# noway/nzcb-circom

Hardware: AMD Instinct MI355X
Metric: PLONK proofs/sec for nzcp_live (~2^21 constraints) at 1/2/4/8 MI355X (higher is better)
Workload: dtype u32 limbs: BN254 Fr/Fq Montgomery, 8x32-bit and 9x29-bit (MSM, NTT twiddles, quotient); 1 GPU; nzcp_live fullProve: NZCPPubIdentity(1,351,0,4,2,4) witness on the GPU (600560 signals) + PLONK proof, n=2^21, nPublic=3, 2970 inputs; domain_size=2097152, n_public=3, n_constraints=1785813, n_vars=1782570, n_additions=1182010, proofs_per_gpu=140, total_proofs=140, parallelism=batch-shard x1 (no collective), proofs_in_flight_per_gpu=5

## Files before the change

include/nzcb_internal.h:

```cpp
#ifndef NZCB_INTERNAL_H
#define NZCB_INTERNAL_H

#include "nzcb.h"

#ifdef __cplusplus
extern "C" {
#endif

int nzcb_ctx_kernel_stats(nzcb_ctx* ctx, int enable, double out[4]);

int nzcb_debug_guard_check(int device, size_t* checked, int* damaged, nzcb_err* err);
int nzcb_debug_guard_selftest(int device, nzcb_err* err);

#define NZCB_FAULT_QUOTIENT 1
#define NZCB_DEBUG_GENERIC_K 2
#define NZCB_FAULT_LANE_ALLOC 3
int nzcb_debug_inject_fault(nzcb_ctx* ctx, int kind);

int nzcb_debug_f29(int device, int op, const uint32_t* in, size_t count, uint32_t* out, nzcb_err* err);

int nzcb_synth_setup(int power, int n_public, int n_inputs, uint64_t seed, uint32_t n_constraints,
                     const uint8_t* tau, int device, uint8_t** zkey_out, size_t* zkey_len, uint8_t** wtns_out,
                     size_t* wtns_len, nzcb_err* err);
#define NZCB_SYNTH_FREE_PUBLIC 1u
int nzcb_synth_setup_ex(int power, int n_public, int n_inputs, uint64_t seed, uint32_t n_constraints, uint32_t flags,
                        const uint8_t* tau, int device, uint8_t** zkey_out, size_t* zkey_len, uint8_t** wtns_out,
                        size_t* wtns_len, nzcb_err* err);
typedef struct nzcb_engine nzcb_engine;
nzcb_engine* nzcb_engine_create(int device, int max_log_ntt, size_t max_msm_points, nzcb_err* err);
void nzcb_engine_destroy(nzcb_engine* e);
int nzcb_engine_ntt(nzcb_engine* e, const uint8_t* in_lem, uint8_t* out_lem, int log_n, int inverse, nzcb_err* err);
int nzcb_engine_msm(nzcb_engine* e, const uint8_t* bases_lem, const uint8_t* scalars, size_t n, int scalars_mont,
                    uint8_t* out_affine, nzcb_err* err);
int nzcb_engine_ntt_dev(nzcb_engine* e, const void* in, void* out, int log_n, int inverse, nzcb_err* err);
int nzcb_engine_msm_dev(nzcb_engine* e, const void* bases, const void* scalars, size_t n, int scalars_mont,
                        uint8_t* out_affine, nzcb_err* err);
int nzcb_engine_time_ntt(nzcb_engine* e, const void* in, void* out, int log_n, int inverse, int reps, double* ms,
                         nzcb_err* err);
int nzcb_engine_random_fr(nzcb_engine* e, void* dev_out, size_t n, uint64_t seed, nzcb_err* err);
int nzcb_engine_fixed_base(nzcb_engine* e, const void* dev_scalars_mont, size_t n, void* dev_out, nzcb_err* err);
int nzcb_engine_lagrange_basis(nzcb_engine* e, const void* dev_ptau, size_t ptau_n, int log_n, void* dev_out,
                               nzcb_err* err);
int nzcb_engine_time_msm(nzcb_engine* e, const void* bases, const void* scalars, size_t n, int scalars_mont, int reps,
                         double* ms, double* acc_ms, nzcb_err* err);
int nzcb_engine_msm_fixed_dev(nzcb_engine* e, const void* bases, size_t n_table, const void* scalars, size_t n,
                              int scalars_mont, uint8_t* out_affine, nzcb_err* err);
int nzcb_engine_msm_table_dev(nzcb_engine* e, const void* bases, size_t n_table, const void* scalars, size_t n,
                              int scalars_mont, int window, int sparse, int fold, uint8_t* out_affine,
                              nzcb_err* err);
int nzcb_engine_msm_sets_dev(nzcb_engine* e, const void* bases, size_t n_table, const void* const* scalars, int sets,
                             size_t n, int scalars_mont, int sparse, uint8_t* out_affine, nzcb_err* err);
int nzcb_engine_time_msm2(nzcb_engine* e, const void* bases, const void* scalars, size_t n, int scalars_mont,
                          int fixed_base, int reps, double* out, nzcb_err* err);
int nzcb_engine_fr_mul(nzcb_engine* e, const uint8_t* a_lem, const uint8_t* b_lem, uint8_t* out_lem, size_t n,
                       int field_q, nzcb_err* err);

int nzcb_engine_g1_lincomb(int device, const uint8_t* points, const uint8_t* scalars, const uint32_t* group_end,
                           size_t groups, uint8_t* out, nzcb_err* err);
int nzcb_engine_verify_batch(const uint8_t* vk, const uint8_t* proofs, const uint8_t* pubs, size_t pub_stride,
                             int n_public, int count, int transcript_public, int device, const uint8_t* seed,
                             int* valid_out, uint8_t* points_out, int* pairing_checks, nzcb_err* err);
int nzcb_debug_verify_batch_timings(double* ms, int cap);

nzcb_r1cs* nzcb_engine_r1cs_create(const uint8_t* r1cs, size_t len, int device, uint32_t long_row_threshold,
                                   int witness_tile, nzcb_err* err);
int nzcb_debug_r1cs_check_timings(double* ms, int cap);

nzcb_p256_key* nzcb_engine_p256_key_create(const uint8_t pub_xy[64], int device, int window, nzcb_err* err);
#define NZCB_P256_OP_ADD 0
#define NZCB_P256_OP_SUB 1
#define NZCB_P256_OP_MUL 2
#define NZCB_P256_OP_SQR 3
#define NZCB_P256_OP_INV 4
int nzcb_debug_p256_field(int device, int op, int field, const uint8_t* a, const uint8_t* b, size_t count,
                          uint8_t* out, nzcb_err* err);
int nzcb_debug_p256_mul2(nzcb_p256_key* k, const uint8_t* u1, const uint8_t* u2, size_t count, uint8_t* out_xy,
                         nzcb_err* err);
int nzcb_debug_p256_timings(double* ms, int cap);

int nzcb_debug_nzcp_decode_timings(double* ms, int cap);

#ifdef __cplusplus
}
#endif
#endif
```

nzcb-circom_amd/csrc/capi_engine.hip:

```cpp
#include <chrono>
#include <cstring>
#include <map>
#include <memory>
#include <mutex>
#include <vector>

#include "../../include/nzcb_internal.h"
#include "engine.h"
#include "lagrange.h"

namespace nzcb {

Engine::Engine(int dev, int max_log_ntt, size_t max_msm_points) : device(dev) {
  NZ_HIP(hipSetDevice(dev));
  NZ_HIP(hipStreamCreateWithFlags(&stream, hipStreamNonBlocking));
  if (max_log_ntt >= 0) ntt_tables.init(max_log_ntt, stream);
  if (max_msm_points) msm_scratch.init(max_msm_points);
}

Engine::~Engine() {
  if (stream) (void)hipStreamDestroy(stream);
}

void set_err(nzcb_err* err, int code, const char* msg) {
// ... 38 lines not shown
  std::vector<uint8_t> h(kGuardBytes);
  int bad = 0;
  for (auto& r : recs) {
    NZ_HIP(hipMemcpy(h.data(), (uint8_t*)r.first + r.second.bytes, kGuardBytes, hipMemcpyDeviceToHost));
    size_t k = 0;
    while (k < kGuardBytes && h[k] == kGuardByte) k++;
    if (k == kGuardBytes) continue;
    bad++;
    if (report && bad <= 8) {
      char line[160];
      std::snprintf(line, sizeof(line), "%sbuffer %p (%zu bytes, device %d): guard byte %zu overwritten",
                    report->empty() ? "" : "; ", r.first, r.second.bytes, r.second.device, k);
      *report += line;
    }
  }
  if (checked) *checked = recs.size();
  return bad;
}

__global__ void k_guard_poke(uint32_t* p, size_t at) {
  if (threadIdx.x == 0) p[at] = 0;
}

}

using namespace nzcb;

struct nzcb_engine {
  Engine eng;
  nzcb_engine(int d, int l, size_t m) : eng(d, l, m) {}
};

#define NZ_GUARD_BEGIN try {
#define NZ_GUARD_END(err)                                   \
  }                                                         \
  catch (const nzcb::Error& e) {                            \
    set_err(err, e.code, e.what());                         \
    return e.code;                                          \
  }                                                         \
  catch (const std::exception& e) {                         \
    set_err(err, NZCB_ERR_INTERNAL, e.what());              \
    return NZCB_ERR_INTERNAL;                               \
  }

__global__ void fe_mul_kernel_r(const Fr* a, const Fr* b, Fr* o, size_t n) {
  size_t i = (size_t)blockIdx.x * blockDim.x + threadIdx.x;
  if (i < n) o[i] = a[i] * b[i];
}
__global__ void fe_mul_kernel_q(const Fq* a, const Fq* b, Fq* o, size_t n) {
  size_t i = (size_t)blockIdx.x * blockDim.x + threadIdx.x;
  if (i < n) o[i] = a[i] * b[i];
}

__global__ void random_fr_kernel(Fr* out, size_t n, uint64_t seed) {
  size_t i = (size_t)blockIdx.x * blockDim.x + threadIdx.x;
  if (i >= n) return;
  uint64_t x = seed ^ (0x9E3779B97F4A7C15ULL * (i + 1));
  Fr v;
  for (int k = 0; k < 4; k++) {
    x += 0x9E3779B97F4A7C15ULL;
    uint64_t z = x;
    z = (z ^ (z >> 30)) * 0xBF58476D1CE4E5B9ULL;
    z = (z ^ (z >> 27)) * 0x94D049BB133111EBULL;
    z ^= z >> 31;
    v.v[2 * k] = (uint32_t)z;
    v.v[2 * k + 1] = (uint32_t)(z >> 32);
  }
  v.v[7] &= 0x1fffffffu;
  out[i] = to_mont(v);
}

static void affine_out(const G1xyzz& r, uint8_t* out) {
  G1Affine a = xyzz_to_affine(r);
  Fq x = a.is_inf() ? Fq::zero() : from_mont(a.x);
  Fq y = a.is_inf() ? Fq::zero() : from_mont(a.y);
  std::memcpy(out, x.v, 32);
  std::memcpy(out + 32, y.v, 32);
}

extern "C" {

const char* nzcb_version(void) { return "nzcb-mi355x 0.1.0 (gfx950)"; }

int nzcb_device_count(void) {
  int n = 0;
  if (hipGetDeviceCount(&n) != hipSuccess) return 0;
  return n;
}

void nzcb_free(void* p) { std::free(p); }

nzcb_engine* nzcb_engine_create(int device, int max_log_ntt, size_t max_msm_points, nzcb_err* err) {
  try {
    return new nzcb_engine(device, max_log_ntt, max_msm_points);
  } catch (const nzcb::Error& e) {
    set_err(err, e.code, e.what());
  } catch (const std::exception& e) {
    set_err(err, NZCB_ERR_INTERNAL, e.what());
  }
  return nullptr;
}

void nzcb_engine_destroy(nzcb_engine* e) { delete e; }

void* nzcb_dev_alloc(size_t bytes) {
  void* p = nullptr;
  if (hipMalloc(&p, bytes) != hipSuccess) return nullptr;
  return p;
}
void* nzcb_dev_alloc_on(int device, size_t bytes) {
  int cur = 0;
  if (hipGetDevice(&cur) != hipSuccess || hipSetDevice(device) != hipSuccess) return nullptr;
  void* p = nullptr;
  if (hipMalloc(&p, bytes) != hipSuccess) p = nullptr;
  (void)hipSetDevice(cur);
  return p;
}
void nzcb_dev_free(void* p) {
  if (p) (void)hipFree(p);
}
int nzcb_memcpy_h2d(void* dst, const void* src, size_t bytes) {
  return hipMemcpy(dst, src, bytes, hipMemcpyHostToDevice) == hipSuccess ? 0 : NZCB_ERR_HIP;
}
int nzcb_memcpy_d2h(void* dst, const void* src, size_t bytes) {
  return hipMemcpy(dst, src, bytes, hipMemcpyDeviceToHost) == hipSuccess ? 0 : NZCB_ERR_HIP;
}
int nzcb_memcpy_d2d(void* dst, const void* src, size_t bytes) {
  if (hipMemcpyAsync(dst, src, bytes, hipMemcpyDeviceToDevice, nullptr) != hipSuccess) return NZCB_ERR_HIP;
  return hipStreamSynchronize(nullptr) == hipSuccess ? 0 : NZCB_ERR_HIP;
}
int nzcb_memcpy_d2d_async(void* dst, const void* src, size_t bytes, void* stream) {
  return hipMemcpyAsync(dst, src, bytes, hipMemcpyDeviceToDevice, (hipStream_t)stream) == hipSuccess ? 0
                                                                                              : NZCB_ERR_HIP;
}

int nzcb_engine_ntt_dev(nzcb_engine* e, const void* in, void* out, int log_n, int inverse, nzcb_err* err) {
  NZ_GUARD_BEGIN
  Engine& g = e->eng;
  NZ_HIP(hipSetDevice(g.device));
  ntt(g.ntt_tables, (const Fr*)in, (Fr*)out, log_n, inverse != 0, g.stream);
  NZ_HIP(hipStreamSynchronize(g.stream));
  return 0;
  NZ_GUARD_END(err)
}

int nzcb_engine_ntt(nzcb_engine* e, const uint8_t* in_lem, uint8_t* out_lem, int log_n, int inverse, nzcb_err* err) {
  NZ_GUARD_BEGIN
  Engine& g = e->eng;
  NZ_HIP(hipSetDevice(g.device));
  size_t n = size_t(1) << log_n;
  DevBuf<Fr> a(n), b(n);
  NZ_HIP(hipMemcpyAsync(a.p, in_lem, n * 32, hipMemcpyHostToDevice, g.stream));
  ntt(g.ntt_tables, a.p, b.p, log_n, inverse != 0, g.stream);
  NZ_HIP(hipMemcpyAsync(out_lem, b.p, n * 32, hipMemcpyDeviceToHost, g.stream));
  NZ_HIP(hipStreamSynchronize(g.stream));
  return 0;
  NZ_GUARD_END(err)
}

int nzcb_engine_time_ntt(nzcb_engine* e, const void* in, void* out, int log_n, int inverse, int reps, double* ms,
                         nzcb_err* err) {
  NZ_GUARD_BEGIN
  Engine& g = e->eng;
  NZ_HIP(hipSetDevice(g.device));
  hipEvent_t e0, e1;
  NZ_HIP(hipEventCreate(&e0));
  NZ_HIP(hipEventCreate(&e1));
  NZ_HIP(hipEventRecord(e0, g.stream));
  for (int i = 0; i < reps; i++) ntt(g.ntt_tables, (const Fr*)in, (Fr*)out, log_n, inverse != 0, g.stream);
  NZ_HIP(hipEventRecord(e1, g.stream));
  NZ_HIP(hipEventSynchronize(e1));
  float t = 0;
  NZ_HIP(hipEventElapsedTime(&t, e0, e1));
  *ms = t / (reps > 0 ? reps : 1);
  (void)hipEventDestroy(e0);
  (void)hipEventDestroy(e1);
  return 0;
  NZ_GUARD_END(err)
}

int nzcb_engine_msm_dev(nzcb_engine* e, const void* bases, const void* scalars, size_t n, int scalars_mont,
                        uint8_t* out_affine, nzcb_err* err) {
  NZ_GUARD_BEGIN
  Engine& g = e->eng;
  NZ_HIP(hipSetDevice(g.device));
  G1xyzz r = msm(g.msm_scratch, (const G1Affine*)bases, (const Fr*)scalars, n, scalars_mont != 0, g.stream);
  affine_out(r, out_affine);
  return 0;
  NZ_GUARD_END(err)
}

int nzcb_engine_msm(nzcb_engine* e, const uint8_t* bases_lem, const uint8_t* scalars, size_t n, int scalars_mont,
                    uint8_t* out_affine, nzcb_err* err) {
  NZ_GUARD_BEGIN
  Engine& g = e->eng;
  NZ_HIP(hipSetDevice(g.device));
  DevBuf<G1Affine> b(n ? n : 1);
  DevBuf<Fr> s(n ? n : 1);
  NZ_HIP(hipMemcpyAsync(b.p, bases_lem, n * 64, hipMemcpyHostToDevice, g.stream));
  NZ_HIP(hipMemcpyAsync(s.p, scalars, n * 32, hipMemcpyHostToDevice, g.stream));
  G1xyzz r = msm(g.msm_scratch, b.p, s.p, n, scalars_mont != 0, g.stream);
  affine_out(r, out_affine);
  return 0;
  NZ_GUARD_END(err)
}

int nzcb_engine_random_fr(nzcb_engine* e, void* dev_out, size_t n, uint64_t seed, nzcb_err* err) {
  NZ_GUARD_BEGIN
  Engine& g = e->eng;
  NZ_HIP(hipSetDevice(g.device));
  hipLaunchKernelGGL(random_fr_kernel, dim3(grid_for(n, 256, 1u << 30)), dim3(256), 0, g.stream, (Fr*)dev_out, n,
                     seed);
  NZ_HIP(hipGetLastError());
  NZ_HIP(hipStreamSynchronize(g.stream));
  return 0;
  NZ_GUARD_END(err)
}

int nzcb_engine_fixed_base(nzcb_engine* e, const void* dev_scalars_mont, size_t n, void* dev_out, nzcb_err* err) {
  NZ_GUARD_BEGIN
  Engine& g = e->eng;
  NZ_HIP(hipSetDevice(g.device));
  launch_fixed_base((const Fr*)dev_scalars_mont, n, (G1Affine*)dev_out, g.stream);
  NZ_HIP(hipStreamSynchronize(g.stream));
  return 0;
  NZ_GUARD_END(err)
}

int nzcb_engine_lagrange_basis(nzcb_engine* e, const void* dev_ptau, size_t ptau_n, int log_n, void* dev_out,
                               nzcb_err* err) {
  NZ_GUARD_BEGIN
  Engine& g = e->eng;
  NZ_HIP(hipSetDevice(g.device));
  lagrange_basis((const G1Affine*)dev_ptau, ptau_n, log_n, (G1Affine*)dev_out, g.stream);
  return 0;
  NZ_GUARD_END(err)
}

int nzcb_engine_time_msm(nzcb_engine* e, const void* bases, const void* scalars, size_t n, int scalars_mont, int reps,
                         double* ms, double* acc_ms, nzcb_err* err) {
  NZ_GUARD_BEGIN
  Engine& g = e->eng;
  NZ_HIP(hipSetDevice(g.device));
  MsmScratch& sc = g.msm_scratch;
  sc.prof = true;
  sc.prof_ms = 0;
  sc.prof_launches = 0;
  auto t0 = std::chrono::steady_clock::now();
  for (int i = 0; i < reps; i++) (void)msm(sc, (const G1Affine*)bases, (const Fr*)scalars, n, scalars_mont != 0, g.stream);
  *ms = std::chrono::duration<double, std::milli>(std::chrono::steady_clock::now() - t0).count() / (reps ? reps : 1);
  *acc_ms = sc.prof_ms / (sc.prof_launches ? sc.prof_launches : 1);
  sc.prof = false;
  return 0;
  NZ_GUARD_END(err)
}

int nzcb_engine_msm_fixed_dev(nzcb_engine* e, const void* bases, size_t n_table, const void* scalars, size_t n,
                              int scalars_mont, uint8_t* out_affine, nzcb_err* err) {
  return nzcb_engine_msm_table_dev(e, bases, n_table, scalars, n, scalars_mont, 0, 0, 0, out_affine, err);
}

int nzcb_engine_msm_table_dev(nzcb_engine* e, const void* bases, size_t n_table, const void* scalars, size_t n,
                              int scalars_mont, int window, int sparse, int fold, uint8_t* out_affine, nzcb_err* err) {
  NZ_GUARD_BEGIN
  Engine& g = e->eng;
  NZ_HIP(hipSetDevice(g.device));
  if (n > n_table) throw Error(NZCB_ERR_ARG, "msm larger than its base table");
  if (window && (window < 16 || window > 20)) throw Error(NZCB_ERR_ARG, "msm table window: 16..20");
  MsmBaseTable t;
  t.build((const G1Affine*)bases, n_table, window ? window : fixed_base_window(), g.stream, fold != 0);
  t.sparse = sparse != 0;
  MsmScratch sc;
  sc.init(n ? n : 1, true);
  G1xyzz r = msm(sc, (const G1Affine*)bases, (const Fr*)scalars, n, scalars_mont != 0, g.stream, &t);
  affine_out(r, out_affine);
  return 0;
  NZ_GUARD_END(err)
}

int nzcb_engine_msm_sets_dev(nzcb_engine* e, const void* bases, size_t n_table, const void* const* scalars, int sets,
                             size_t n, int scalars_mont, int sparse, uint8_t* out_affine, nzcb_err* err) {
  NZ_GUARD_BEGIN
  Engine& g = e->eng;
  NZ_HIP(hipSetDevice(g.device));
  if (n > n_table) throw Error(NZCB_ERR_ARG, "msm larger than its base table");
  if (sets < 1 || sets > 3 || !scalars) throw Error(NZCB_ERR_ARG, "msm sets: 1..3 scalar vectors");
  MsmBaseTable t;
  t.build((const G1Affine*)bases, n_table, lagrange_window(), g.stream);
  t.sparse = sparse != 0;
  MsmScratch sc;
  sc.init(n ? n : 1, true, 3, false);
  G1xyzz r[3] = {G1xyzz::inf(), G1xyzz::inf(), G1xyzz::inf()};
  msm_enqueue_sets(sc, (const Fr* const*)scalars, sets, n, scalars_mont != 0, g.stream, &t);
  msm_finish_sets(sc, g.stream, r);
  for (int k = 0; k < sets; k++) affine_out(r[k], out_affine + 64 * k);
  return 0;
  NZ_GUARD_END(err)
}

int nzcb_engine_time_msm2(nzcb_engine* e, const void* bases, const void* scalars, size_t n, int scalars_mont,
                          int fixed_base, int reps, double* out, nzcb_err* err) {
  NZ_GUARD_BEGIN
  Engine& g = e->eng;
  NZ_HIP(hipSetDevice(g.device));
  std::unique_ptr<MsmBaseTable> t;
  std::unique_ptr<MsmScratch> own;
// ... 180 lines not shown
```

nzcb-circom_amd/csrc/f29.h:

```cpp
#pragma once
#include "field.h"

namespace nzcb {

struct F29 {
  uint32_t v[9];
};

struct Fq29 {
  static constexpr uint32_t MASK = (1u << 29) - 1;
  static constexpr uint32_t INV = 0x04866389u;
  static constexpr uint32_t P[9] = {0x187cfd47u, 0x010460b6u, 0x1c72a34fu, 0x02d522d0u, 0x1585d978u,
                                    0x02db40c0u, 0x00a6e141u, 0x0e5c2634u, 0x0030644eu};
  static constexpr uint32_t K2[9] = {0x30f9fa8eu, 0x2208c16cu, 0x38e5469du, 0x25aa45a0u, 0x2b0bb2efu,
                                     0x25b68180u, 0x214dc281u, 0x3cb84c67u, 0x0060c89bu};
  static constexpr uint32_t K4[9] = {0x21f3f51cu, 0x241182dau, 0x31ca8d3bu, 0x2b548b42u, 0x361765dfu,
                                     0x2b6d0301u, 0x229b8503u, 0x397098cfu, 0x00c19138u};
  static constexpr uint32_t K6[9] = {0x32edefaau, 0x261a4447u, 0x2aafd3d9u, 0x30fed0e4u, 0x212318cfu,
                                     0x31238483u, 0x23e94785u, 0x3628e537u, 0x012259d5u};
  static constexpr uint32_t K8[9] = {0x23e7ea38u, 0x282305b5u, 0x23951a77u, 0x36a91686u, 0x2c2ecbbfu,
                                     0x36da0604u, 0x25370a07u, 0x32e1319fu, 0x01832272u};
  static constexpr uint32_t ONE[9] = {0x157ccc21u, 0x141c2758u, 0x185230d3u, 0x014c0419u, 0x0aa36fb9u,
                                      0x1d4240ceu, 0x11d54c07u, 0x052ac7a8u, 0x000dc836u};
  static constexpr uint32_t C256[9] = {0x058f0d9du, 0x1aea1c6eu, 0x11c2cf74u, 0x11d651ebu, 0x1462c0a7u,
// ... 407 lines not shown
  F29 r;
#pragma unroll
  for (int i = 0; i < 9; i++) r.v[i] = a.v[i] + (b.v[i] << 1);
  norm29(r);
  return r;
}

NZ_HD F29 sub29_nn(const F29& a, const F29& b, const uint32_t (&K)[9]) {
  F29 r;
#pragma unroll
  for (int i = 0; i < 9; i++) r.v[i] = a.v[i] + K[i] - b.v[i];
  return r;
}
NZ_HD F29 neg4p29_nn(const F29& y) {
  F29 r;
#pragma unroll
  for (int i = 0; i < 9; i++) r.v[i] = Fq29::K4[i] - y.v[i];
  return r;
}
NZ_HD F29 neg29_nn(const F29& y) {
  F29 r;
#pragma unroll
  for (int i = 0; i < 9; i++) r.v[i] = Fq29::K2[i] - y.v[i];
  return r;
}
struct Fq29W {
  static constexpr uint32_t K10[9] = {0x34e1e4c6u, 0x2a2bc722u, 0x3c7a6115u, 0x3c535c27u, 0x373a7eafu,
                                      0x3c908785u, 0x2684cc89u, 0x2f997e07u, 0x01e3eb0fu};
  static constexpr uint32_t K6W[9] = {0x92edefaau, 0x861a4444u, 0x8aafd3d6u, 0x90fed0e1u, 0x812318ccu,
                                      0x91238480u, 0x83e94782u, 0x9628e534u, 0x012259d2u};
};
NZ_HD F29 sub2x29(const F29& a, const F29& b, const F29& c) {
  F29 r;
#pragma unroll
  for (int i = 0; i < 9; i++) r.v[i] = a.v[i] + Fq29W::K6W[i] - b.v[i] - (c.v[i] << 1);
  norm29(r);
  return r;
}

NZ_HD F29 neg4p29(const F29& y) {
  F29 r;
#pragma unroll
  for (int i = 0; i < 9; i++) r.v[i] = Fq29::K4[i] - y.v[i];
  norm29(r);
  return r;
}

NZ_HD F29 neg29(const F29& y) {
  F29 r;
  r.v[0] = Fq29::P[0] + (1u << 29) - y.v[0];
#pragma unroll
  for (int i = 1; i < 8; i++) r.v[i] = Fq29::P[i] + (1u << 29) - 1u - y.v[i];
  r.v[8] = Fq29::P[8] - 1u - y.v[8];
  norm29(r);
  return r;
}

NZ_HD bool is0p29(const F29& x) {
  uint32_t o0 = 0, op = 0;
#pragma unroll
  for (int i = 0; i < 9; i++) {
    o0 |= x.v[i];
    op |= x.v[i] ^ Fq29::P[i];
  }
  return o0 == 0 || op == 0;
}

NZ_HD bool is0p29_fast(const F29& x) {
  if (x.v[0] != 0u && x.v[0] != Fq29::P[0]) return false;
  return is0p29(x);
}

template <class Par>
NZ_HD F29 split29(const Fe<Par>& x) {
  F29 r;
#pragma unroll
  for (int i = 0; i < 9; i++) {
    const int bit = 29 * i, limb = bit >> 5, sh = bit & 31;
    uint64_t w = x.v[limb];
    if (limb + 1 < 8) w |= (uint64_t)x.v[limb + 1] << 32;
    r.v[i] = (uint32_t)(w >> sh) & Fq29::MASK;
  }
  return r;
}
NZ_HD Fq join29(const F29& x) {
  Fq r;
#pragma unroll
  for (int i = 0; i < 8; i++) r.v[i] = 0;
#pragma unroll
  for (int i = 0; i < 9; i++) {
    const int bit = 29 * i, limb = bit >> 5, sh = bit & 31;
    const uint64_t w = (uint64_t)x.v[i] << sh;
    r.v[limb] |= (uint32_t)w;
    if (limb + 1 < 8) r.v[limb + 1] |= (uint32_t)(w >> 32);
  }
  return r;
}

NZ_HD Fr join_fr29(const F29& t) {
  Fr r;
#pragma unroll
  for (int i = 0; i < 8; i++) r.v[i] = 0;
#pragma unroll
  for (int i = 0; i < 9; i++) {
    const int bit = 29 * i, limb = bit >> 5, sh = bit & 31;
    const uint64_t w = (uint64_t)t.v[i] << sh;
    r.v[limb] |= (uint32_t)w;
    if (limb + 1 < 8) r.v[limb + 1] |= (uint32_t)(w >> 32);
  }
  return reduce_once(r);
}
NZ_HD Fr canon_fr29(const F29& x) {
  const uint32_t q = x.v[8] / (Fr29::P[8] + 1u);
  F29 y;
  int64_t carry = 0;
#pragma unroll
  for (int l = 0; l < 9; l++) {
    const int64_t t = (int64_t)x.v[l] + carry - (int64_t)((uint64_t)q * Fr29::P[l]);
    y.v[l] = l < 8 ? ((uint32_t)t & Fr29::MASK) : (uint32_t)t;
    carry = t >> 29;
  }
  return join_fr29(y);
}
NZ_HD Fr mul_fr29(const Fr& a, const F29& w29) {
  return join_fr29(mul29<Fr29>(split29(a), w29));
}

NZ_HD Fr from_mont_fr29(const Fr& a) {
  using Q = Fr29;
  const F29 x = split29(a);
  uint32_t m[9];
  F29 r;
  uint64_t acc = 0;
#pragma unroll
  for (int i = 0; i < 9; i++) {
    acc += (uint64_t)x.v[i] << 5;
#pragma unroll
    for (int j = 0; j < i; j++) mad29c(acc, m[j], Q::P[i - j]);
    m[i] = ((uint32_t)acc * Q::INV) & Q::MASK;
    mad29c(acc, m[i], Q::P[0]);
    acc >>= 29;
  }
#pragma unroll
  for (int i = 9; i < 17; i++) {
#pragma unroll
    for (int j = i - 8; j < 9; j++) mad29c(acc, m[j], Q::P[i - j]);
    r.v[i - 9] = (uint32_t)acc & Q::MASK;
    acc >>= 29;
  }
  r.v[8] = (uint32_t)acc;
  return join_fr29(r);
}

NZ_HD F29 fr_to261(const Fr& x) {
  const F29 r = split29(x);
  F29 o;
  o.v[0] = (r.v[0] << 5) & Fr29::MASK;
#pragma unroll
  for (int l = 1; l < 9; l++) o.v[l] = ((r.v[l] << 5) & Fr29::MASK) | (r.v[l - 1] >> 24);
  return o;
}
NZ_HD F29 add3_29(const F29& a, const F29& b, const F29& c) {
  F29 r;
#pragma unroll
  for (int l = 0; l < 9; l++) r.v[l] = a.v[l] + b.v[l] + c.v[l];
  norm29(r);
  return r;
}
NZ_HD Fr fr_from261(const F29& x) { return join_fr29(mul29<Fr29>(x, f29_const(Fr29::C256))); }

NZ_HD Fq to_fq256(const F29& x) { return reduce_once(join29(mul29(x, f29_const(Fq29::C256)))); }

struct alignas(16) Xyzz29 {
  F29 X, Y, ZZ, ZZZ;
};

NZ_HD Xyzz29 mdbl29(const F29& x, const F29& y) {
  Xyzz29 r;
  F29 U;
#pragma unroll
  for (int i = 0; i < 9; i++) U.v[i] = y.v[i] << 1;
  const F29 V = sqr29(U);
  const F29 W = mul29(U, V);
  const F29 S = mul29(x, V);
  const F29 xx = sqr29(x);
  F29 M;
#pragma unroll
  for (int i = 0; i < 9; i++) M.v[i] = xx.v[i] * 3u;
  norm29(M);
  const F29 t = add29(S, S);
  r.X = sub29(sqr29(M), t, Fq29::K4);
  const F29 d = sub29(S, r.X, Fq29::K8);
  r.Y = sub29(mul29(M, d), mul29(W, y), Fq29::K2);
  r.ZZ = V;
  r.ZZZ = W;
  return r;
}

NZ_HD bool is_inf29(const Xyzz29& a) {
  uint32_t z = 0;
#pragma unroll
  for (int i = 0; i < 9; i++) z |= a.ZZ.v[i];
  return z == 0;
}

NZ_HD Xyzz29 dbl29(const Xyzz29& p) {
  Xyzz29 r;
  F29 U;
#pragma unroll
  for (int i = 0; i < 9; i++) U.v[i] = p.Y.v[i] << 1;
  const F29 V = sqr29(U);
  const F29 W = mul29(U, V);
  const F29 S = mul29(p.X, V);
  const F29 xx = sqr29(p.X);
  F29 M;
#pragma unroll
  for (int i = 0; i < 9; i++) M.v[i] = xx.v[i] * 3u;
  norm29(M);
  r.X = sub29(sqr29(M), add29(S, S), Fq29::K4);
  r.Y = sub29(mul29(M, sub29(S, r.X, Fq29::K8)), mul29(W, p.Y), Fq29::K2);
  r.ZZ = mul29(V, p.ZZ);
  r.ZZZ = mul29(W, p.ZZZ);
  return r;
}

NZ_HD Xyzz29 add29(const Xyzz29& p, const Xyzz29& q) {
  if (is_inf29(p)) return q;
  if (is_inf29(q)) return p;
  F29 U1, U2, S1, S2, PP, RR, PPP, Q, Z12, ZZZ12;
  mul29x2<Fq29>(p.X, q.ZZ, q.X, p.ZZ, U1, U2);
  mul29x2<Fq29>(p.Y, q.ZZZ, q.Y, p.ZZZ, S1, S2);
  const F29 P = sub29(U2, U1, Fq29::K2);
  const F29 R = sub29(S2, S1, Fq29::K2);
  sqr29x2(P, R, PP, RR);
  mul29x2<Fq29>(P, PP, U1, PP, PPP, Q);
  mul29x2<Fq29>(p.ZZ, q.ZZ, p.ZZZ, q.ZZZ, Z12, ZZZ12);
  Xyzz29 r;
  mul29x2<Fq29>(Z12, PP, ZZZ12, PPP, r.ZZ, r.ZZZ);
  if (is0p29(r.ZZ)) {
    if (is0p29(RR)) return dbl29(p);
    Xyzz29 inf = r;
#pragma unroll
    for (int i = 0; i < 9; i++) inf.ZZ.v[i] = 0;
    return inf;
  }
  r.X = sub29(RR, add2x29(PPP, Q), Fq29::K6);
  F29 y1, y2;
  mul29x2<Fq29>(R, sub29(Q, r.X, Fq29::K8), S1, PPP, y1, y2);
  r.Y = sub29(y1, y2, Fq29::K2);
  return r;
}

}
```

nzcb-circom_amd/csrc/f29_check.hip:

```cpp
#include "../../include/nzcb_internal.h"
#include "common.h"
#include "f29.h"

namespace nzcb {
namespace {

constexpr int kIn[7] = {0, 27, 54, 18, 36, 18, 36};
constexpr int kOut[7] = {0, 9, 18, 9, 18, 18, 9};

__device__ __forceinline__ F29 ld(const uint32_t* p) {
  F29 r;
#pragma unroll
  for (int i = 0; i < 9; i++) r.v[i] = p[i];
  return r;
}
__device__ __forceinline__ void st(uint32_t* p, const F29& x) {
#pragma unroll
  for (int i = 0; i < 9; i++) p[i] = x.v[i];
}

template <int OP>
__global__ void __launch_bounds__(64) k_f29_check(const uint32_t* __restrict__ in, uint32_t* __restrict__ out,
                                                  size_t count) {
  const size_t t = (size_t)blockIdx.x * 64 + threadIdx.x;
  if (t >= count) return;
  const uint32_t* a = in + t * kIn[OP];
  uint32_t* o = out + t * kOut[OP];
  if constexpr (OP == 1) {
    st(o, mul_shoup(ld(a), ld(a + 9), ld(a + 18)));
  } else if constexpr (OP == 2) {
    F29 r1, r2;
    mul_shoup_x2(ld(a), ld(a + 9), ld(a + 18), ld(a + 27), ld(a + 36), ld(a + 45), r1, r2);
    st(o, r1);
    st(o + 9, r2);
  } else if constexpr (OP == 3) {
    st(o, mul29<Fq29>(ld(a), ld(a + 9)));
  } else if constexpr (OP == 4) {
    F29 r1, r2;
    mul29x2<Fr29>(ld(a), ld(a + 9), ld(a + 18), ld(a + 27), r1, r2);
    st(o, r1);
    st(o + 9, r2);
  } else if constexpr (OP == 5) {
    F29 r1, r2;
    sqr29x2(ld(a), ld(a + 9), r1, r2);
    st(o, r1);
    st(o + 9, r2);
  } else {
    st(o, mul2sum29(ld(a), ld(a + 9), ld(a + 18), ld(a + 27)));
  }
}

template <int OP>
void launch(const uint32_t* in, uint32_t* out, size_t count) {
  hipLaunchKernelGGL(k_f29_check<OP>, dim3((unsigned)((count + 63) / 64)), dim3(64), 0, nullptr, in, out, count);
}

}
}

using namespace nzcb;

extern "C" int nzcb_debug_f29(int device, int op, const uint32_t* in, size_t count, uint32_t* out, nzcb_err* err) {
  auto fail = [&](int code, const std::string& m) {
    if (err) {
      err->code = code;
      std::snprintf(err->msg, sizeof(err->msg), "%s", m.c_str());
    }
    return code;
  };
  if (op < 1 || op > 6 || (count && (!in || !out)) || count > (size_t(1) << 24))
    return fail(NZCB_ERR_ARG, "f29 check: op 1..6, count <= 2^24");
  try {
    if (count) {
      NZ_HIP(hipSetDevice(device));
      DevBuf<uint32_t> din(count * kIn[op]), dout(count * kOut[op]);
      NZ_HIP(hipMemcpy(din.p, in, count * kIn[op] * 4, hipMemcpyHostToDevice));
      switch (op) {
        case 1: launch<1>(din.p, dout.p, count); break;
        case 2: launch<2>(din.p, dout.p, count); break;
        case 3: launch<3>(din.p, dout.p, count); break;
        case 4: launch<4>(din.p, dout.p, count); break;
        case 5: launch<5>(din.p, dout.p, count); break;
        default: launch<6>(din.p, dout.p, count); break;
      }
      NZ_HIP(hipGetLastError());
      NZ_HIP(hipMemcpy(out, dout.p, count * kOut[op] * 4, hipMemcpyDeviceToHost));
    }
    if (err) err->code = 0;
    return 0;
  } catch (const Error& e) {
    return fail(e.code, e.what());
  } catch (const std::exception& e) {
    return fail(NZCB_ERR_INTERNAL, e.what());
  }
}
```

nzcb-circom_amd/csrc/ntt.h:

```cpp
#pragma once
#include "f29.h"
#include "common.h"

namespace nzcb {

Fr fr_root_of_unity(int k);

struct NttTables {
  int max_log = 0;
  struct Tw {
    F29 w, ws;
  };
  DevBuf<Tw> fwd29, inv29;
  DevBuf<uint32_t> scratch29;
  void init(int max_log, hipStream_t st);
};

struct NttIo {
  size_t in_len = ~size_t(0);
  const F29* in_f = nullptr;
  size_t fold_len = 0, fold_n = 0;
  F29 fold_f = {};
  const F29* out_f = nullptr;
  bool out_f_has_scale = false;
  size_t out_limit = ~size_t(0);
  uint32_t* out_flags = nullptr;
};

void ntt(const NttTables& t, const Fr* in, Fr* out, int log_n, bool inverse, hipStream_t st,
         const Fr* scale = nullptr, const NttIo* io = nullptr, uint32_t* scratch29 = nullptr);

}
```

nzcb-circom_amd/csrc/ntt.hip:

```cpp
#include "ntt.h"

#include <vector>

namespace nzcb {

static constexpr int kTile = 1024;

Fr fr_root_of_unity(int k) {
  Fr w;
  const uint32_t w28[8] = {0x725b19f0u, 0x9bd61b6eu, 0x41112ed4u, 0x402d111eu,
                           0x8ef62abcu, 0x00e0a7ebu, 0xa58a7e85u, 0x2a3c09f0u};
  for (int i = 0; i < 8; i++) w.v[i] = w28[i];
  w = to_mont(w);
  for (int j = 28; j > k; j--) w = sqr(w);
  return w;
}

__device__ __forceinline__ uint32_t bit_rev(uint32_t x, int bits) {
  return bits ? (__brev(x) >> (32 - bits)) : 0u;
}

__global__ void __launch_bounds__(256)
ntt_table_kernel(Fr* __restrict__ out, const Fr* __restrict__ lo, const Fr* __restrict__ hi, size_t count) {
  size_t i = (size_t)blockIdx.x * blockDim.x + threadIdx.x;
  if (i >= count) return;
  out[i] = lo[i & 2047] * hi[i >> 11];
}

__global__ void __launch_bounds__(256)
ntt_stage_table_kernel(Fr* __restrict__ out, const Fr* __restrict__ full, int L, size_t count) {
  size_t i = (size_t)blockIdx.x * blockDim.x + threadIdx.x;
  if (i >= count) return;
  int g = 63 - __clzll((unsigned long long)(i + 1));
  size_t k = i + 1 - ((size_t)1 << g);
  out[i] = full[k << (L - g - 1)];
}

__global__ void __launch_bounds__(256) ntt_tw29_kernel(NttTables::Tw* __restrict__ out, const Fr* __restrict__ tw,
                                                       size_t count) {
  size_t i = (size_t)blockIdx.x * blockDim.x + threadIdx.x;
  if (i >= count) return;
  Fr m = tw[i];
#pragma unroll
  for (int k = 0; k < 5; k++) m = m + m;
  NttTables::Tw t;
  t.w = split29(from_mont(tw[i]));
  t.ws = mul_lo261(split29(m), f29_const(Fr29::NINV));
  out[i] = t;
}

void NttTables::init(int L, hipStream_t st) {
  max_log = L;
  if (L > 8) scratch29.alloc((size_t)9 << L);
  const size_t half = L >= 1 ? (size_t(1) << (L - 1)) : 1;
  const size_t total = (size_t(1) << L) - 1;
  DevBuf<Fr> stage(total ? total : 1);
  fwd29.alloc(total ? total : 1);
  inv29.alloc(total ? total : 1);
  DevBuf<Fr> full(half);
  for (int dir = 0; dir < 2; dir++) {
    Fr w = fr_root_of_unity(L);
    if (dir) w = inverse(w);
    size_t nlo = half < 2048 ? half : 2048;
    size_t nhi = (half + 2047) / 2048;
    std::vector<Fr> lo(2048, Fr::one()), hi(nhi, Fr::one());
    for (size_t i = 1; i < nlo; i++) lo[i] = lo[i - 1] * w;
    Fr w2048 = pow_u64(w, 2048);
    for (size_t i = 1; i < nhi; i++) hi[i] = hi[i - 1] * w2048;
    DevBuf<Fr> dlo(2048), dhi(nhi);
    NZ_HIP(hipMemcpyAsync(dlo.p, lo.data(), 2048 * sizeof(Fr), hipMemcpyHostToDevice, st));
    NZ_HIP(hipMemcpyAsync(dhi.p, hi.data(), nhi * sizeof(Fr), hipMemcpyHostToDevice, st));
    hipLaunchKernelGGL(ntt_table_kernel, dim3(grid_for(half, 256, 1u << 30)), dim3(256), 0, st, full.p, dlo.p, dhi.p,
                       half);
    if (total) {
      hipLaunchKernelGGL(ntt_stage_table_kernel, dim3(grid_for(total, 256, 1u << 30)), dim3(256), 0, st,
                         stage.p, full.p, L, total);
      hipLaunchKernelGGL(ntt_tw29_kernel, dim3(grid_for(total, 256, 1u << 30)), dim3(256), 0, st,
                         dir ? inv29.p : fwd29.p, stage.p, total);
    }
    NZ_HIP(hipGetLastError());
    NZ_HIP(hipStreamSynchronize(st));
  }
}


__device__ __forceinline__ int tile_slot(int e) {
  return e ^ ((((e >> 5) & 3) << 3) | ((e >> 5) & 7));
}
__device__ __forceinline__ F29 tile_ld(const uint32_t* sl, int e) {
  const int p = tile_slot(e);
  F29 x;
#pragma unroll
  for (int l = 0; l < 9; l++) x.v[l] = sl[l * kTile + p];
  return x;
}
__device__ __forceinline__ void tile_st(uint32_t* sl, int e, const F29& x) {
  const int p = tile_slot(e);
#pragma unroll
  for (int l = 0; l < 9; l++) sl[l * kTile + p] = x.v[l];
}
__device__ __forceinline__ F29 add_nn29(const F29& a, const F29& b) {
  F29 r;
#pragma unroll
  for (int l = 0; l < 9; l++) r.v[l] = a.v[l] + b.v[l];
  return r;
}
__device__ __forceinline__ F29 tw_mul(const F29& x, const NttTables::Tw& w) { return mul_shoup(x, w.w, w.ws); }
__device__ __forceinline__ void tw_mul2(const F29& x, const NttTables::Tw& w, const F29& y, const NttTables::Tw& v,
                                        F29& r1, F29& r2) {
  mul_shoup_x2(x, w.w, w.ws, y, v.w, v.ws, r1, r2);
}
__device__ __forceinline__ F29 sub4r_nn29(const F29& a, const F29& b) {
  F29 r;
#pragma unroll
  for (int l = 0; l < 9; l++) r.v[l] = a.v[l] + Fr29::K4[l] - b.v[l];
  return r;
}

template <bool IN29, bool OUT29>
__global__ void __launch_bounds__(kTile / 4)
ntt29_pass_kernel(const Fr* in, const F29* in29, Fr* out, F29* out29, const NttTables::Tw* __restrict__ tw, int L, int s,
                  int q, int logC, F29 scale29, int do_scale, NttIo io, int sparse4) {
  constexpr int T = kTile / 4;
  __shared__ uint32_t sl[9 * kTile];
  const int C = 1 << logC;
  const int rows = 1 << q;
  const int n_el = rows << logC;
  const int tid = threadIdx.x;
  const size_t t = blockIdx.x;
  size_t base = 0, c0 = 0, lo0 = 0;
  if (!IN29) {
    c0 = t << logC;
    for (int e = tid; e < n_el; e += T) {
      const int j = e >> logC, c = e & (C - 1);
      const size_t src = ((size_t)bit_rev((uint32_t)j, q) << (L - q)) + c0 + c;
      F29 x;
#pragma unroll
      for (int l = 0; l < 9; l++) x.v[l] = 0;
      if (src < io.in_len) {
        x = split29(in[src]);
        if (src < io.fold_len) {
          const F29 hi = mul29<Fr29>(split29(in[src + io.fold_n]), io.fold_f);
#pragma unroll
          for (int l = 0; l < 9; l++) x.v[l] += hi.v[l];
          if (!io.in_f) {
            norm29(x);
            x = split29(canon_fr29(x));
          }
        }
        if (io.in_f) x = mul29<Fr29>(x, io.in_f[src]);
        if (do_scale) x = mul29<Fr29>(x, scale29);
      }
      tile_st(sl, e, x);
    }
  } else {
    const size_t groups_lo = ((size_t)1 << s) >> logC;
    const size_t hi = t / groups_lo;
    lo0 = (t % groups_lo) << logC;
    base = (hi << (s + q)) + lo0;
    for (int e = tid; e < n_el; e += T) {
      const int j = e >> logC, c = e & (C - 1);
      tile_st(sl, e, in29[base + ((size_t)j << s) + c]);
    }
  }
  __syncthreads();
  const int nbf = n_el >> 1;
  const bool first = !IN29;
  int st = 0;
  if (sparse4 && blockIdx.x != 0) {
    for (int e = tid; e < n_el; e += T) {
      const int j = e >> logC;
      if (j & 3) tile_st(sl, e, tile_ld(sl, ((j & ~3) << logC) + (e & (C - 1))));
    }
    __syncthreads();
    st = 2;
  } else if (q & 1) {
    const int g = s;
    const NttTables::Tw* __restrict__ twg = tw + (((size_t)1 << g) - 1);
#pragma unroll
    for (int u = 0; u < 2; u++) {
      const int b = tid + u * T;
      if (b >= nbf) continue;
      const int c = b & (C - 1);
      const int j0 = b >> logC;
      const int i0 = ((2 * j0) << logC) + c, i1 = ((2 * j0 + 1) << logC) + c;
      const size_t k = first ? 0 : (lo0 + c);
      const F29 x0 = tile_ld(sl, i0);
      const F29 x1 = tile_ld(sl, i1);
      const F29 tt = g ? tw_mul(x1, twg[k]) : x1;
      F29 y0 = add_nn29(x0, tt), y1 = sub4r_nn29(x0, tt);
      norm29(y0);
      norm29(y1);
      tile_st(sl, i0, y0);
      tile_st(sl, i1, y1);
    }
    __syncthreads();
    st = 1;
  }
  const int ngroups = n_el >> 2;
#pragma unroll 1
  for (; st < q; st += 2) {
    const int h = 1 << st;
    const int g = s + st;
    const NttTables::Tw* __restrict__ twa = tw + (((size_t)1 << g) - 1);
    const NttTables::Tw* __restrict__ twb = tw + (((size_t)1 << (g + 1)) - 1);
    const int b = tid;
    if (b < ngroups) {
      const int c = b & (C - 1);
      const int pr = b >> logC;
      const int low = pr & (h - 1);
      const int j = ((pr >> st) << (st + 2)) | low;
      const size_t ka = first ? (size_t)low : (((size_t)low << s) + lo0 + c);
      const size_t kc = first ? (size_t)(low + h) : (((size_t)(low + h) << s) + lo0 + c);
      const int i0 = (j << logC) + c, i1 = ((j + h) << logC) + c, i2 = ((j + 2 * h) << logC) + c,
                i3 = ((j + 3 * h) << logC) + c;
      F29 t1 = tile_ld(sl, i1), t3 = tile_ld(sl, i3);
      if (g) {
        const NttTables::Tw wa = twa[ka];
        F29 p1, p3;
        tw_mul2(t1, wa, t3, wa, p1, p3);
        t1 = p1;
        t3 = p3;
      }
      const F29 x0 = tile_ld(sl, i0), x2 = tile_ld(sl, i2);
      const F29 y0 = add_nn29(x0, t1), y1 = sub4r_nn29(x0, t1);
      const F29 y2 = add_nn29(x2, t3), y3 = sub4r_nn29(x2, t3);
      F29 u2, u3;
      const NttTables::Tw wb = twb[ka], wc = twb[kc];
      tw_mul2(y2, wb, y3, wc, u2, u3);
      F29 z0 = add_nn29(y0, u2), z2 = sub4r_nn29(y0, u2), z1 = add_nn29(y1, u3), z3 = sub4r_nn29(y1, u3);
      norm29(z0);
      norm29(z1);
      norm29(z2);
      norm29(z3);
      tile_st(sl, i0, z0);
      tile_st(sl, i1, z1);
      tile_st(sl, i2, z2);
      tile_st(sl, i3, z3);
    }
    __syncthreads();
  }
  auto store = [&](size_t dst, const F29& x) {
    if (OUT29) {
      out29[dst] = x;
    } else {
      const Fr v = io.out_f ? join_fr29(mul29<Fr29>(x, io.out_f[dst])) : canon_fr29(x);
      if (io.out_flags && dst >= io.out_limit && !v.is_zero()) atomicOr(io.out_flags, 1u);
      out[dst] = v;
    }
  };
  if (first) {
    for (int e = tid; e < n_el; e += T) {
      const int j = e & (rows - 1), c = e >> q;
      const size_t dst = ((size_t)bit_rev((uint32_t)(c0 + c), L - q) << q) + j;
      store(dst, tile_ld(sl, (j << logC) + c));
    }
  } else {
    for (int e = tid; e < n_el; e += T) {
      const int j = e >> logC, c = e & (C - 1);
      store(base + ((size_t)j << s) + c, tile_ld(sl, e));
    }
  }
}

static void ntt29_passes(const Fr* in, Fr* out, const NttTables::Tw* tw, int L, const F29& sc29, int do_scale,
                         const NttIo& io, hipStream_t st, F29* scr) {
  constexpr int T = kTile / 4;
  const int q1 = L < 8 ? L : 8;
  const int cols = 1 << (L - q1);
  int logC1 = 0;
  while ((1 << (logC1 + 1)) <= cols && ((1 << (q1 + logC1 + 1)) <= kTile)) logC1++;
  const size_t tiles = (size_t)cols >> logC1;
  const int sparse4 = L >= 2 && q1 >= 2 && !(q1 & 1) &&
                      io.in_len <= ((size_t)1 << (L - 2)) + ((size_t)1 << logC1);
  if (q1 == L) {
    hipLaunchKernelGGL((ntt29_pass_kernel<false, false>), dim3((unsigned)tiles), dim3(T), 0, st, in,
                       (const F29*)nullptr, out, (F29*)nullptr, tw, L, 0, q1, logC1, sc29, do_scale, io, sparse4);
    NZ_HIP(hipGetLastError());
    return;
  }
  hipLaunchKernelGGL((ntt29_pass_kernel<false, true>), dim3((unsigned)tiles), dim3(T), 0, st, in,
                     (const F29*)nullptr, (Fr*)nullptr, scr, tw, L, 0, q1, logC1, sc29, do_scale, io, sparse4);
  NZ_HIP(hipGetLastError());
  int s = q1;
  while (s < L) {
    const int q = (L - s) < 8 ? (L - s) : 8;
    int logC = 0;
    while (logC + 1 <= s && (1 << (q + logC + 1)) <= kTile) logC++;
    const size_t ntiles = ((size_t)1 << (L - s - q)) * (((size_t)1 << s) >> logC);
    if (s + q == L)
      hipLaunchKernelGGL((ntt29_pass_kernel<true, false>), dim3((unsigned)ntiles), dim3(T), 0, st,
                         (const Fr*)nullptr, (const F29*)scr, out, (F29*)nullptr, tw, L, s, q, logC, sc29, 0, io, 0);
    else
      hipLaunchKernelGGL((ntt29_pass_kernel<true, true>), dim3((unsigned)ntiles), dim3(T), 0, st,
                         (const Fr*)nullptr, (const F29*)scr, (Fr*)nullptr, scr, tw, L, s, q, logC, sc29, 0, io, 0);
    NZ_HIP(hipGetLastError());
    s += q;
  }
}

void ntt(const NttTables& t, const Fr* in, Fr* out, int L, bool inverse_dir, hipStream_t st, const Fr* scale,
         const NttIo* iop, uint32_t* scratch29) {
  const NttIo io = iop ? *iop : NttIo();
  if (L > t.max_log) throw Error(NZCB_ERR_ARG, "ntt size exceeds table");
  if (in == out) throw Error(NZCB_ERR_ARG, "ntt requires in != out");
  F29* scr = (F29*)(scratch29 ? scratch29 : t.scratch29.p);
  if (L > 8 && !scratch29 && t.scratch29.n < ((size_t)9 << L)) throw Error(NZCB_ERR_INTERNAL, "ntt: no scratch");
  const NttTables::Tw* tw = inverse_dir ? t.inv29.p : t.fwd29.p;
  Fr sc = Fr::one();
  int do_scale = 0;
  if (inverse_dir && !io.out_f_has_scale) {
    Fr two = Fr::one() + Fr::one();
    sc = inverse(pow_u64(two, (uint64_t)L));
    do_scale = 1;
  }
  if (scale) {
    sc = do_scale ? sc * *scale : *scale;
    do_scale = 1;
  }
  for (int k = 0; k < 5; k++) sc = sc + sc;
  ntt29_passes(in, out, tw, L, split29(sc), do_scale, io, st, scr);
}

}
```

nzcb-circom_amd/csrc/prover.h:

```cpp
#pragma once
#include <chrono>
#include <functional>
#include <memory>
#include <string>
#include <vector>

#include "engine.h"
#include "zkey.h"

namespace nzcb {

struct AddRec {
  uint32_t ai, bi, dst, pad;
  Fr ac, bc;
};

struct MsmShard {
  static constexpr int kSlots = 3;
  int device = 0;
  size_t lo = 0, hi = 0;
  size_t llo = 0, lhi = 0;
  MsmBaseTable table, ltable;
  std::unique_ptr<MsmScratch> sc[kSlots];
  DevBuf<Fr> scal[kSlots];
  hipStream_t st[kSlots] = {nullptr, nullptr, nullptr};
  ~MsmShard();
};

struct Prover {
  uint32_t n = 0, n4 = 0, nVars = 0, nPublic = 0, nAdditions = 0, nConstraints = 0, nWit = 0;
  int power = 0;
  Fr k1, k2, wn, w2;
  std::vector<uint32_t> add_level_start;
  bool transcript_public = true;
  std::function<void(const std::string&)> log;

  std::unique_ptr<Engine> eng;
  static constexpr int kSlots = 3;
  std::unique_ptr<MsmScratch> msc[kSlots];
  hipStream_t aux[kSlots] = {nullptr, nullptr, nullptr};
  hipEvent_t ready[kSlots] = {nullptr, nullptr, nullptr};
  bool slot_split[kSlots] = {false, false, false};
  bool slot_lag[kSlots] = {false, false, false};
  hipEvent_t side_ready = nullptr, side_done = nullptr, pows_done = nullptr;
  ~Prover();
  DevBuf<G1Affine> ptau;
  MsmBaseTable ptab;
  DevBuf<G1Affine> ltau;
  MsmBaseTable ltab;
  bool lcommit = false;
  DevBuf<Fr> qm, ql, qr, qo, qc;
  DevBuf<Fr> sigma;
  DevBuf<Fr> sig_h;
  DevBuf<Fr> q_h;
  DevBuf<Fr> w_h;
  DevBuf<Fr> lagrange;
  DevBuf<uint32_t> amap, bmap, cmap;
  DevBuf<AddRec> adds;
  DevBuf<Fr> root_lo, root_hi;
  DevBuf<Fr> x_lo;
  DevBuf<Fr> g_lo, g_hi, gi_lo, gi_hi;
  DevBuf<F29> g29, gi29;
  Fr zh_inv[4];
  DevBuf<Fr> cq, cs, cl;
  bool quot3 = false;
  DevBuf<Fr> cq3, cs3, cl3;
  DevBuf<F29> tw3, itw3;
  Fr d3[3];
  Fr sig_top[3][4];
  DevBuf<Fr> wit;
  DevBuf<Fr> wtns_in;
  DevBuf<Fr> A, B, C, Z;
  DevBuf<Fr> pol_a, pol_b, pol_c, pol_z;
  DevBuf<Fr> A4, B4, C4, Z4, T, Tz, t;
  DevBuf<Fr> pol_r, pol_wxi, pol_wxiw;
  DevBuf<Fr> blind;
  DevBuf<Fr> scan_tmp;
  DevBuf<Fr> lin_tab;
  size_t lin_qn = 0;
  Fr* lin_tile_pows(int k);
  std::vector<Fr> lin_host;
  DevBuf<Fr> eval_part;
  DevBuf<F29> eval_pw;
  DevBuf<uint32_t> flags;
  std::vector<Fr> host_part;
  DevBuf<uint32_t> ntt_scr2;
  Fr* top_host = nullptr;
  static constexpr int kMbFlags = 24, kMbTotals = 25, kMbEvals = 27, kMbEvalMax = 8;
  size_t mb_apub = 0, mb_pubw = 0, mb_words = 0;

  int lane_id = 0;
  int fault = 0;
  double tm[11] = {0};
  bool prof_gpu = false;
  std::vector<std::pair<hipEvent_t, hipEvent_t>> span_ev;
  std::vector<int> span_kind;
  size_t spans_used = 0;
  size_t span_begin(int kind, hipStream_t s);
  void span_end(size_t i, hipStream_t s);
  void span_totals(double* msm_ms, double* ntt_ms);

  Prover(const uint8_t* zkey, size_t len, int device);
  Prover(const Prover& primary, int lane);
  void set_msm_devices(const std::vector<int>& devices);
  std::vector<std::unique_ptr<MsmShard>> shards;
  size_t own_hi = 0, own_lhi = 0;
  nzcb_msm_send_fn split_send = nullptr;
  nzcb_msm_gather_fn split_gather = nullptr;
  void* split_user = nullptr;
  int split_world = 1;
  size_t split_own = 0, split_own_l = 0;
  void set_msm_split(int world, size_t own_points, size_t own_lagrange, nzcb_msm_send_fn send,
                     nzcb_msm_gather_fn gather, void* user);
  void prove(const uint8_t* witness, size_t n_witness, const uint8_t* blinding, uint8_t* proof_out,
             uint8_t* pub_out, bool witness_on_device = false);

 private:
  hipStream_t st() const { return eng->stream; }
  void init_slots();
  void alloc_workspace();
  void to4t(const Fr* evals, Fr* coefs, Fr* evals4, const int* bidx, int nb, hipStream_t s = nullptr);
  void to4t_coefs(const Fr* evals, Fr* coefs, const int* bidx, int nb, hipStream_t s, uint32_t* scr = nullptr);
  void to4t_evals4(const Fr* coefs, Fr* evals4, int nb, hipStream_t s, uint32_t* scr = nullptr);
  void round3_quot3(const Fr& beta, const Fr& gamma, const Fr& alpha, hipStream_t s);
  void launch_gate_check(hipStream_t s);
  void copy_tops(hipStream_t s);
  void commit_start(int slot, const Fr* scalars, size_t len, const MsmBaseTable* tab = nullptr,
                    const G1Affine* bases = nullptr, bool on_main = false);
  G1Affine commit_finish(int slot);
  void commit_start_abc(size_t len);
  void commit_finish_abc(G1Affine& a, G1Affine& b, G1Affine& c);
  void eval_many(int np, const Fr* const* polys, const size_t* lens, const Fr* xs, Fr* out,
                 const std::function<void()>& overlap = nullptr);
  void div_pol1(const Fr* src, size_t m, int tab, const Fr& p0_adjust, Fr* dst, uint32_t flag_bit);
  void lin_tables(int k, const Fr& d, hipStream_t s);
  double ms_since(std::chrono::steady_clock::time_point t0);
  double msm_ms = 0, ntt_ms = 0;
};

}
```

nzcb-circom_amd/csrc/prover.hip:

```cpp
#include <rocprofiler-sdk-roctx/roctx.h>
#include "lagrange.h"
#include "prover.h"
#include "transcript.h"

#include <cstring>
#include <cerrno>
#include <string>
#include <sys/random.h>

#include "keccak.h"

namespace nzcb {

static constexpr int kT = 256;
static constexpr uint32_t kZeroRef = 0xffffffffu;

__global__ void k_wit_to_mont(const Fr* __restrict__ in, Fr* __restrict__ out, size_t n) {
  size_t i = (size_t)blockIdx.x * blockDim.x + threadIdx.x;
  if (i >= n) return;
  out[i] = (i == 0) ? Fr::zero() : to_mont(in[i]);
}

__global__ void k_additions(const AddRec* __restrict__ recs, uint32_t count, Fr* __restrict__ wit) {
  uint32_t i = blockIdx.x * blockDim.x + threadIdx.x;
// ... 374 lines not shown
  const Fr f = F[blockIdx.x] * inv_d;
  const size_t base = (size_t)blockIdx.x * kTileN + threadIdx.x;
#pragma unroll
  for (int k = 0; k < kPer; k++) {
    const size_t i = base + (size_t)k * kT;
    if (i < m) x[i] = x[i] * f;
  }
}

struct LinTab {
  Fr P[kT + 1];
  Fr Pinv[kT + 1];
  Fr dp[kPer + 1];
};
static_assert(sizeof(LinTab) % sizeof(Fr) == 0, "LinTab is stored as Fr words");

template <bool kWrite>
__global__ void __launch_bounds__(kT)
k_lin_tile(const Fr* __restrict__ src, size_t m, const LinTab* __restrict__ tab, const Fr* __restrict__ carry,
           Fr* __restrict__ out) {
  __shared__ uint32_t stg[kStageWords];
  __shared__ Fr sh[kT / 64];
  const int tid = threadIdx.x;
  const size_t base = (size_t)blockIdx.x * kTileN;
  Fr x[kPer];
  stage_in([&](size_t g) { return src[g + 1]; }, base, m - 1, stg, x);
  const Fr d = tab->dp[1];
  Fr y = Fr::zero();
#pragma unroll
  for (int j = kPer - 1; j >= 0; j--) {
    y = x[j] + d * y;
    x[j] = y;
  }
  Fr total;
  Fr ex = block_sum_excl_suffix(y * tab->P[tid], sh, total);
  if (!kWrite) {
    if (tid == 0) out[blockIdx.x] = total;
    return;
  }
  if (carry) ex = ex + carry[blockIdx.x + 1] * tab->P[kT];
  const Fr next = ex * tab->Pinv[tid + 1];
#pragma unroll
  for (int j = 0; j < kPer; j++) x[j] = x[j] + tab->dp[kPer - j] * next;
  stage_out(x, base, m, stg, out);
}

__global__ void k_pow_tiles(Fr D, Fr Di, int count, Fr* __restrict__ Q, Fr* __restrict__ Qinv) {
  const int T = blockIdx.x * blockDim.x + threadIdx.x;
  if (T >= count) return;
  Fr a = Fr::one(), b = Fr::one(), pa = D, pb = Di;
  for (int e = T; e; e >>= 1) {
    if (e & 1) {
      a = a * pa;
      b = b * pb;
    }
    pa = sqr(pa);
    pb = sqr(pb);
  }
  Q[T] = a;
  Qinv[T] = b;
}

__global__ void __launch_bounds__(1024) k_tile_heads(Fr* __restrict__ h, int m, const Fr* __restrict__ Q,
                                                     const Fr* __restrict__ Qinv) {
  __shared__ Fr sh[1024 / 64];
  const int tid = threadIdx.x;
  const int per = (m + 1023) / 1024;
  const int t0 = min(tid * per, m), t1 = min(t0 + per, m);
  Fr run = Fr::zero();
  for (int T = t0; T < t1; T++) run = run + h[T] * Q[T];
  Fr suf = block_scan_excl<true, AddOp, 1024>(run, sh, nullptr);
  for (int T = t1 - 1; T >= t0; T--) {
    suf = suf + h[T] * Q[T];
    h[T] = suf * Qinv[T];
  }
  if (tid == 0) h[m] = Fr::zero();
}

__global__ void k_stride4(const Fr* __restrict__ src, size_t n, Fr* __restrict__ dst) {
  const size_t i = (size_t)blockIdx.x * blockDim.x + threadIdx.x;
  if (i < n) dst[i] = src[4 * i];
}

struct QArgs {
  Fr beta, gamma, alpha, alpha2, bk1, bk2;
  Fr zhinv[4];
};

__global__ void __launch_bounds__(kT)
k_quotient_coset(const Fr* __restrict__ A, const Fr* __restrict__ B, const Fr* __restrict__ C,
                 const Fr* __restrict__ Z, const Fr* __restrict__ cq, const Fr* __restrict__ cs,
                 const Fr* __restrict__ cl, uint32_t npub, const Fr* __restrict__ Apub, size_t n,
                 const Fr* __restrict__ xlo, const Fr* __restrict__ xhi, QArgs q, Fr* __restrict__ T) {
  const size_t n4 = 4 * n;
  size_t i = (size_t)blockIdx.x * blockDim.x + threadIdx.x;
  if (i >= n4) return;
  const Fr a = A[i], b = B[i], c = C[i];
  const Fr x = xlo[i & 4095] * xhi[i >> 12];
  Fr gate = a * b * cq[i] + a * cq[n4 + i] + b * cq[2 * n4 + i] + c * cq[3 * n4 + i] + cq[4 * n4 + i];
  for (uint32_t j = 0; j < npub; j++) gate = gate - cl[j * n4 + i] * Apub[j];
  const Fr z = Z[i];
  const Fr bx = q.beta * x;
  Fr num = (a + bx + q.gamma) * (b + q.bk1 * x + q.gamma);
  num = num * (c + q.bk2 * x + q.gamma) * z;
  Fr den = (a + q.beta * cs[i] + q.gamma) * (b + q.beta * cs[n4 + i] + q.gamma);
  den = den * (c + q.beta * cs[2 * n4 + i] + q.gamma) * Z[(i + 4) & (n4 - 1)];
  const Fr e4 = (z - Fr::one()) * cl[i] * q.alpha2;
  T[i] = (gate + q.alpha * (num - den) + e4) * q.zhinv[i & 3];
}

constexpr uint32_t kQ29MaxPub = 8;

static bool quot3_enabled() {
  static const bool on = [] {
    const char* e = std::getenv("NZCB_QUOT3");
    return !(e && e[0] == '0');
  }();
  return on;
}
struct QArgs29 {
  F29 beta, bk1, bk2, alpha2, zhinv[4];
  F29 gamma, negone;
  int k23;
  F29 alpha;
};

template <int K>
__device__ __forceinline__ F29 q29_pi_chunk(const Fr* __restrict__ cl, const Fr* __restrict__ Apub, uint32_t j0,
                                            size_t n4, size_t i) {
  F29 pa[K], pb[K];
#pragma unroll
  for (int k = 0; k < K; k++) {
    pa[k] = split29(cl[(size_t)(j0 + k) * n4 + i]);
    pb[k] = split29(neg(Apub[j0 + k]));
  }
  return mulsum29<Fr29, K>(pa, pb);
}

__device__ __forceinline__ F29 q29_pi(const Fr* __restrict__ cl, const Fr* __restrict__ Apub, uint32_t j0,
                                      uint32_t cnt, size_t n4, size_t i) {
  switch (cnt) {
    case 1: return q29_pi_chunk<1>(cl, Apub, j0, n4, i);
    case 2: return q29_pi_chunk<2>(cl, Apub, j0, n4, i);
    case 3: return q29_pi_chunk<3>(cl, Apub, j0, n4, i);
    default: return q29_pi_chunk<4>(cl, Apub, j0, n4, i);
  }
}

template <bool THREE>
__global__ void __launch_bounds__(kT) __attribute__((amdgpu_waves_per_eu(4, 8)))
k_quotient_coset29(const Fr* __restrict__ A, const Fr* __restrict__ B, const Fr* __restrict__ C,
                   const Fr* __restrict__ Z, const Fr* __restrict__ cq, const Fr* __restrict__ cs,
                   const Fr* __restrict__ cl, uint32_t npub, const Fr* __restrict__ Apub, size_t n,
                   const Fr* __restrict__ xlo, const Fr* __restrict__ xhi, QArgs29 q, Fr* __restrict__ T) {
  const size_t n4 = (THREE ? 3 : 4) * n;
  size_t i = (size_t)blockIdx.x * blockDim.x + threadIdx.x;
  if (i >= n4) return;
  size_t ix, izw;
  int cj;
  if (THREE) {
    const int lg = __ffsll((long long)n) - 1;
    const size_t j = i >> lg, m = i & (n - 1);
    ix = 4 * m + j;
    izw = j * n + ((m + 1) & (n - 1));
    cj = (int)j;
  } else {
    ix = i;
    izw = (i + 4) & (n4 - 1);
    cj = (int)(i & 3);
  }
  const F29 a = split29(A[i]), b = split29(B[i]), c = split29(C[i]), z = split29(Z[i]);
  F29 gate;
  {
    const F29 ga[4] = {mul29<Fr29>(a, b), a, b, c};
    const F29 gb[4] = {split29(cq[i]), split29(cq[n4 + i]), split29(cq[2 * n4 + i]), split29(cq[3 * n4 + i])};
    gate = add29(mulsum29<Fr29, 4>(ga, gb), split29(cq[4 * n4 + i]));
  }
  if (npub > 0) gate = add29(gate, q29_pi(cl, Apub, 0, npub < 4 ? npub : 4, n4, i));
  if (npub > 4) gate = add29(gate, q29_pi(cl, Apub, 4, npub - 4, n4, i));
  const F29 x = mul29<Fr29>(split29(xlo[ix & 4095]), split29(xhi[ix >> 12]));
  const F29 bx = mul29<Fr29>(q.beta, x);
  const F29 bx2 = q.k23 ? add29(bx, bx) : mul29<Fr29>(q.bk1, x);
  const F29 bx3 = q.k23 ? add29(bx2, bx) : mul29<Fr29>(q.bk2, x);
  const F29 f1 = add29(add29(a, bx), q.gamma);
  const F29 f2 = add29(add29(b, bx2), q.gamma);
  const F29 f3 = add29(add29(c, bx3), q.gamma);
  const F29 num = mul29<Fr29>(mul29<Fr29>(mul29<Fr29>(f1, f2), f3), z);
  const F29 g1 = add29(add29(a, mul29<Fr29>(q.beta, split29(cs[i]))), q.gamma);
  const F29 g2 = add29(add29(b, mul29<Fr29>(q.beta, split29(cs[n4 + i]))), q.gamma);
  const F29 g3 = add29(add29(c, mul29<Fr29>(q.beta, split29(cs[2 * n4 + i]))), q.gamma);
  const F29 den = mul29<Fr29>(mul29<Fr29>(mul29<Fr29>(g1, g2), g3), split29(Z[izw]));
  const F29 pa[2] = {q.alpha, q.alpha2};
  const F29 pb[2] = {sub29(num, den, Fr29::K2), mul29<Fr29>(add29(z, q.negone), split29(cl[i]))};
  const F29 S = add29(gate, mulsum29<Fr29, 2>(pa, pb));
  T[i] = join_fr29(mul29<Fr29>(S, q.zhinv[cj]));
}

__global__ void __launch_bounds__(kT)
k_gate_h(const Fr* __restrict__ A, const Fr* __restrict__ B, const Fr* __restrict__ C, const Fr* __restrict__ qh,
         size_t n, uint32_t npub, uint32_t* __restrict__ flags) {
  const size_t m = (size_t)blockIdx.x * blockDim.x + threadIdx.x;
  if (m >= n) return;
  const Fr a = A[m], b = B[m], c = C[m];
  Fr g = qh[m] * a * b + qh[n + m] * a + qh[2 * n + m] * b + qh[3 * n + m] * c + qh[4 * n + m];
  if (m < npub) g = g - a;
  if (!g.is_zero()) atomicOr(flags, 1u);
}

struct T3Args {
  Fr c0[6], c1[6], c2[6], q3[6];
  Fr i4, two_over_d, inv_d2;
};
__global__ void __launch_bounds__(kT)
k_t_combine(const Fr* __restrict__ V, size_t n, T3Args a, Fr* __restrict__ t) {
  const size_t k = (size_t)blockIdx.x * blockDim.x + threadIdx.x;
  if (k >= n) return;
  Fr v0 = V[k], v1 = V[n + k], v2 = V[2 * n + k];
  if (k < 6) {
    v0 = v0 - a.c0[k];
    v1 = v1 - a.c1[k];
    v2 = v2 - a.c2[k];
  }
  const Fr sm = v0 + v2, dl = v0 - v2, im = dl * a.i4, v12 = v1 + v1;
  t[k] = sm + v12 - im;
  t[n + k] = dl * a.two_over_d;
  t[2 * n + k] = (sm - v12 + im) * a.inv_d2;
  if (k < 6) t[3 * n + k] = a.q3[k];
}

__global__ void k_root_n(Fr* __restrict__ out, const Fr* __restrict__ rlo, const Fr* __restrict__ rhi, size_t n) {
  const size_t i = (size_t)blockIdx.x * blockDim.x + threadIdx.x;
  if (i < n) out[i] = root4(rlo, rhi, 4 * i);
}

__global__ void k_fault_bump(Fr* x) {
  if (threadIdx.x == 0) x[0] = x[0] + Fr::one();
}

__global__ void k_dbl_pow(Fr* __restrict__ x, size_t m, int e) {
  size_t i = (size_t)blockIdx.x * blockDim.x + threadIdx.x;
  if (i >= m) return;
  Fr v = x[i];
  for (int k = 0; k < e; k++) v = v + v;
  x[i] = v;
}

static F29 f29_exp(Fr v, int extra) {
  for (int k = 0; k < extra; k++) v = v + v;
  return split29(v);
}

static constexpr int kEvalMax = 8;
static constexpr int kEvalBits = 16;
struct EvalSet {
  const Fr* p[kEvalMax];
  uint64_t len[kEvalMax];
  Fr x[kEvalMax];
  Fr x4096[kEvalMax];
  F29 x29[kEvalMax];
  F29 y29[kEvalMax];
  int np;
  int nbits;
};

__device__ __forceinline__ F29 fr29_operand_dev(Fr c) {
#pragma unroll
  for (int k = 0; k < 5; k++) c = c + c;
  return split29(c);
}

static constexpr int kEvalChunk2 = 16;

__global__ void __launch_bounds__(kT) k_eval_pows(EvalSet es, F29* __restrict__ pw, Fr* __restrict__ pw2) {
  const int j = blockIdx.x, t = threadIdx.x;
  Fr a = Fr::one(), q = es.x[j];
  for (int e = t; e; e >>= 1) {
    if (e & 1) a = a * q;
    q = q * q;
  }
  pw[(size_t)j * kT + t] = fr29_operand_dev(a);
  if (t < es.nbits) {
    Fr z = es.x4096[j];
    for (int k = 0; k < t; k++) z = z * z;
    pw2[j * kEvalBits + t] = z;
  }
}

__device__ __forceinline__ Fr block_sum_fr(const Fr& v, Fr* sh) {
  Fr x = v;
#pragma unroll
  for (int m = 32; m >= 1; m >>= 1) x = x + shfl_fr(x, (int)(threadIdx.x & 63) ^ m);
  if ((threadIdx.x & 63) == 0) sh[threadIdx.x >> 6] = x;
  __syncthreads();
  Fr t = sh[0];
#pragma unroll
  for (int k = 1; k < kT / 64; k++) t = t + sh[k];
  __syncthreads();
  return t;
}

template <int NP>
__global__ void __launch_bounds__(kT) k_eval_multi(EvalSet es, const F29* __restrict__ pw, const Fr* __restrict__ pw2,
                                                   Fr* __restrict__ partial, int nblocks) {
  static_assert(NP <= kEvalMax && kEvalMax <= 4 * (kT / 64), "one 16-lane group per point");
  __shared__ Fr sh[kT / 64];
  __shared__ Fr bpow[kEvalMax];
  __shared__ Fr bsum[kEvalMax];
  {
    const int l = (int)(threadIdx.x & 63), k = l & 15, j = 4 * (int)(threadIdx.x >> 6) + (l >> 4);
    Fr f = Fr::one();
    if (j < NP && k < es.nbits && ((blockIdx.x >> k) & 1u)) f = pw2[j * kEvalBits + k];
    for (int m = 8; m >= 1; m >>= 1) f = f * shfl_fr(f, l ^ m);
    if (j < NP && k == 0) bpow[j] = f;
  }
  const size_t s = (size_t)blockIdx.x * kT * kEvalChunk2 + threadIdx.x;
  F29 acc[NP];
#pragma unroll
  for (int j = 0; j < NP; j++)
#pragma unroll
    for (int l = 0; l < 9; l++) acc[j].v[l] = 0;
  for (int m = kEvalChunk2 - 1; m >= 0; m--) {
    const size_t i = s + (size_t)m * kT;
#pragma unroll
    for (int j = 0; j < NP; j++)
      if (i < es.len[j]) {
        const F29 t = mul29<Fr29>(acc[j], es.y29[j]), c = split29(es.p[j][i]);
#pragma unroll
        for (int l = 0; l < 9; l++) acc[j].v[l] = t.v[l] + c.v[l];
      }
  }
#pragma unroll
  for (int j = 0; j < NP; j++) {
    const Fr r = block_sum_fr(join_fr29(mul29<Fr29>(acc[j], pw[(size_t)j * kT + threadIdx.x])), sh);
    if (threadIdx.x == 0) bsum[j] = r;
  }
  if (threadIdx.x < NP) partial[(size_t)threadIdx.x * nblocks + blockIdx.x] = bsum[threadIdx.x] * bpow[threadIdx.x];
}

__global__ void __launch_bounds__(kT) k_eval_sum(const Fr* __restrict__ partial, int nblocks, Fr* __restrict__ out) {
  __shared__ Fr sh[kT / 64];
  const int j = blockIdx.x;
  Fr acc = Fr::zero();
  for (int b = (int)threadIdx.x; b < nblocks; b += kT) acc = acc + partial[(size_t)j * nblocks + b];
  const Fr r = block_sum_fr(acc, sh);
  if (threadIdx.x == 0) {
    host_put(out + j, r);
    host_put_done();
  }
// ... 173 lines not shown
      DevBuf<G1Affine> part(lcnt);
      NZ_HIP(hipMemcpyPeerAsync(part.p, sh->device, ltau.p + sh->llo, eng->device, lcnt * sizeof(G1Affine),
                                sh->st[0]));
      sh->ltable.build(part.p, lcnt, lagrange_window(), sh->st[0]);
      sh->ltable.sparse = lagrange_sparse();
      NZ_HIP(hipStreamSynchronize(sh->st[0]));
    }
    shards.push_back(std::move(sh));
  }
  NZ_HIP(hipSetDevice(eng->device));
}

double Prover::ms_since(std::chrono::steady_clock::time_point t0) {
  return std::chrono::duration<double, std::milli>(std::chrono::steady_clock::now() - t0).count();
}

Prover::Prover(const uint8_t* zkey_bytes, size_t len, int device) {
  GuardScope guards;
  Zkey z = parse_zkey(zkey_bytes, len);
  n = z.domainSize;
  n4 = 4 * n;
  power = z.power;
  nVars = z.nVars;
  nPublic = z.nPublic;
  nAdditions = z.nAdditions;
  nConstraints = z.nConstraints;
  if (nAdditions > nVars) throw Error(NZCB_ERR_FORMAT, "nAdditions > nVars");
  nWit = nVars - nAdditions;
  k1 = z.k1;
  k2 = z.k2;
  wn = fr_root_of_unity(power);
  w2 = fr_root_of_unity(2);
  eng.reset(new Engine(device, power + 2, 0));
  init_slots();
  hipStream_t s = st();
  auto up = [&](auto& buf, const Section& sec) {
    using T = typename std::remove_reference<decltype(*buf.p)>::type;
    buf.alloc(sec.len / sizeof(T) ? sec.len / sizeof(T) : 1);
    if (sec.len) NZ_HIP(hipMemcpyAsync(buf.p, sec.p, sec.len, hipMemcpyHostToDevice, s));
  };
  up(ptau, z.ptau);
  ptab.build(ptau.p, ptau.n, fixed_base_window(), s, true);
  lcommit = lagrange_commit_enabled() && ptau.n >= (size_t)n + 2;
  if (lcommit) {
    ltau.alloc((size_t)n + 2);
    lagrange_basis(ptau.p, ptau.n, power, ltau.p, s);
    ltab.build(ltau.p, ltau.n, lagrange_window(), s);
    ltab.sparse = lagrange_sparse();
  }
  up(qm, z.qm);
  up(ql, z.ql);
  up(qr, z.qr);
  up(qo, z.qo);
  up(qc, z.qc);
  up(sigma, z.sigma);
  sig_h.alloc((size_t)3 * n);
  w_h.alloc(n);
  for (int k = 0; k < 3; k++)
    hipLaunchKernelGGL(k_stride4, dim3(grid_for(n, kT, 1u << 30)), dim3(kT), 0, s, sigma.p + (size_t)k * 5 * n + n,
                       (size_t)n, sig_h.p + (size_t)k * n);
  NZ_HIP(hipGetLastError());
  up(lagrange, z.lagrange);
  up(amap, z.amap);
  up(bmap, z.bmap);
  up(cmap, z.cmap);
  {
    std::vector<uint32_t> level(nAdditions, 0);
    std::vector<AddRec> recs(nAdditions);
    uint32_t maxlev = 0;
    for (uint32_t k = 0; k < nAdditions; k++) {
      const uint8_t* p = z.additions.p + (size_t)k * 72;
      AddRec r;
      std::memcpy(&r.ai, p, 4);
      std::memcpy(&r.bi, p + 4, 4);
      std::memcpy(r.ac.v, p + 8, 32);
      std::memcpy(r.bc.v, p + 40, 32);
      r.dst = nWit + k;
      r.pad = 0;
      uint32_t lv = 0;
      for (uint32_t* ref : {&r.ai, &r.bi}) {
        if (*ref >= nVars) *ref = kZeroRef;
        else if (*ref >= nWit) {
          uint32_t kk = *ref - nWit;
          if (kk >= k) *ref = kZeroRef;
          else lv = std::max(lv, level[kk] + 1);
        }
      }
      level[k] = lv;
      maxlev = std::max(maxlev, lv);
      recs[k] = r;
    }
    std::vector<uint32_t> cnt(maxlev + 2, 0);
    for (uint32_t k = 0; k < nAdditions; k++) cnt[level[k] + 1]++;
    for (uint32_t l = 1; l < cnt.size(); l++) cnt[l] += cnt[l - 1];
    add_level_start.assign(cnt.begin(), cnt.end());
    std::vector<AddRec> sorted(nAdditions);
    std::vector<uint32_t> cur(cnt.begin(), cnt.end());
    for (uint32_t k = 0; k < nAdditions; k++) sorted[cur[level[k]]++] = recs[k];
    adds.alloc(nAdditions ? nAdditions : 1);
    if (nAdditions)
      NZ_HIP(hipMemcpyAsync(adds.p, sorted.data(), nAdditions * sizeof(AddRec), hipMemcpyHostToDevice, s));
    NZ_HIP(hipStreamSynchronize(s));
  }
  Fr w4 = fr_root_of_unity(power + 2);
  size_t nlo = 4096, nhi = (n4 + 4095) / 4096;
  const Fr one = Fr::one();
  auto table = [&](DevBuf<Fr>& out, size_t cnt, const Fr& base, const Fr& scale) {
    out.alloc(cnt);
    hipLaunchKernelGGL(k_root_table, dim3(grid_for(cnt, kT)), dim3(kT), 0, s, out.p, base, scale, cnt);
    NZ_HIP(hipGetLastError());
  };
  table(root_lo, nlo, w4, one);
  table(root_hi, nhi, pow_u64(w4, 4096), one);
  hipLaunchKernelGGL(k_root_n, dim3(grid_for(n, kT, 1u << 30)), dim3(kT), 0, s, w_h.p, root_lo.p, root_hi.p,
                     (size_t)n);
  NZ_HIP(hipGetLastError());
  const Fr g = fr_small(5), gi = inverse(g);
  table(x_lo, nlo, w4, g);
  table(g_lo, nlo, g, one);
  table(g_hi, nhi, pow_u64(g, 4096), one);
  table(gi_lo, nlo, gi, one);
  table(gi_hi, nhi, pow_u64(gi, 4096), one);
  quot3 = quot3_enabled() && nPublic <= kQ29MaxPub && power >= 6;
  {
    const Fr two = one + one;
    g29.alloc((size_t)n + 8);
    hipLaunchKernelGGL(k_factor29_table, dim3(grid_for((size_t)n + 8, kT, 1u << 30)), dim3(kT), 0, s, g29.p, g_lo.p,
                       g_hi.p, one, (size_t)n + 8);
    if (!quot3) {
      gi29.alloc(n4);
      hipLaunchKernelGGL(k_factor29_table, dim3(grid_for(n4, kT, 1u << 30)), dim3(kT), 0, s, gi29.p, gi_lo.p,
                         gi_hi.p, inverse(pow_u64(two, (uint64_t)power + 2)), (size_t)n4);
    }
    NZ_HIP(hipGetLastError());
  }
  {
    Fr gn = pow_u64(g, n), w4n = pow_u64(w4, n), p = gn;
    for (int k = 0; k < 4; k++) {
      zh_inv[k] = inverse(p - one);
      p = p * w4n;
    }
  }
  alloc_workspace();
  if (quot3) {
    q_h.alloc((size_t)5 * n);
    const DevBuf<Fr>* qs[5] = {&qm, &ql, &qr, &qo, &qc};
    for (int k = 0; k < 5; k++)
      hipLaunchKernelGGL(k_stride4, dim3(grid_for(n, kT, 1u << 30)), dim3(kT), 0, s, qs[k]->p + n, (size_t)n,
                         q_h.p + (size_t)k * n);
    NZ_HIP(hipGetLastError());
  }
  if (quot3) {
    const size_t nhi3 = (n + 4095) / 4096;
    tw3.alloc((size_t)3 * n);
    itw3.alloc((size_t)3 * n);
    const Fr inv4n = inverse(fr_small(n4));
    DevBuf<Fr> lo, hi;
    for (int j = 0; j < 3; j++) {
      const Fr cj = g * pow_u64(w4, (uint64_t)j), cji = inverse(cj);
      d3[j] = pow_u64(cj, n);
      table(lo, nlo, cj, one);
      table(hi, nhi3, pow_u64(cj, 4096), one);
      hipLaunchKernelGGL(k_factor29_table, dim3(grid_for(n, kT, 1u << 30)), dim3(kT), 0, s, tw3.p + (size_t)j * n,
                         lo.p, hi.p, one, (size_t)n);
      NZ_HIP(hipStreamSynchronize(s));
      table(lo, nlo, cji, one);
      table(hi, nhi3, pow_u64(cji, 4096), one);
      hipLaunchKernelGGL(k_factor29_table, dim3(grid_for(n, kT, 1u << 30)), dim3(kT), 0, s, itw3.p + (size_t)j * n,
                         lo.p, hi.p, inv4n, (size_t)n);
      NZ_HIP(hipGetLastError());
      NZ_HIP(hipStreamSynchronize(s));
    }
    for (int k = 0; k < 3; k++)
      NZ_HIP(hipMemcpy(sig_top[k], sigma.p + (size_t)k * 5 * n + (n - 4), 4 * sizeof(Fr), hipMemcpyDeviceToHost));
  }
  if (quot3) {
    const uint32_t nl = nPublic > 0 ? nPublic : 1;
    const size_t n3 = (size_t)3 * n;
    cq3.alloc(5 * n3);
    cs3.alloc(3 * n3);
    cl3.alloc(nl * n3);
    auto coset3 = [&](const Fr* coefs, Fr* out) {
      for (int j = 0; j < 3; j++) {
        NttIo io;
        io.in_len = n;
        io.in_f = tw3.p + (size_t)j * n;
        ntt(eng->ntt_tables, coefs, out + (size_t)j * n, power, false, s, nullptr, &io);
      }
    };
    const DevBuf<Fr>* qs[5] = {&qm, &ql, &qr, &qo, &qc};
    for (int k = 0; k < 5; k++) coset3(qs[k]->p, cq3.p + (size_t)k * n3);
    for (int k = 0; k < 3; k++) coset3(sigma.p + (size_t)k * 5 * n, cs3.p + (size_t)k * n3);
    for (uint32_t j = 0; j < nl; j++) coset3(lagrange.p + (size_t)j * 5 * n, cl3.p + (size_t)j * n3);
    NZ_HIP(hipGetLastError());
    auto scale = [&](Fr* p, size_t m, int e) {
      hipLaunchKernelGGL(k_dbl_pow, dim3(grid_for(m, kT, 1u << 30)), dim3(kT), 0, s, p, m, e);
    };
    scale(cq3.p, n3, 10);
    scale(cq3.p + n3, 3 * n3, 5);
    scale(cl3.p, (size_t)nl * n3, 5);
    scale(x_lo.p, nlo, 5);
    NZ_HIP(hipGetLastError());
  } else {
    const uint32_t nl = nPublic > 0 ? nPublic : 1;
    cq.alloc((size_t)5 * n4);
    cs.alloc((size_t)3 * n4);
    cl.alloc((size_t)nl * n4);
    auto coset_eval = [&](const Fr* coefs, Fr* out) {
      NttIo io;
      io.in_len = n;
      io.in_f = g29.p;
      ntt(eng->ntt_tables, coefs, out, power + 2, false, s, nullptr, &io);
    };
    const DevBuf<Fr>* qs[5] = {&qm, &ql, &qr, &qo, &qc};
    for (int k = 0; k < 5; k++) coset_eval(qs[k]->p, cq.p + (size_t)k * n4);
    for (int k = 0; k < 3; k++) coset_eval(sigma.p + (size_t)k * 5 * n, cs.p + (size_t)k * n4);
    for (uint32_t j = 0; j < nl; j++) coset_eval(lagrange.p + (size_t)j * 5 * n, cl.p + (size_t)j * n4);
    NZ_HIP(hipGetLastError());
    if (nPublic <= kQ29MaxPub) {
      auto scale = [&](Fr* p, size_t m, int e) {
        hipLaunchKernelGGL(k_dbl_pow, dim3(grid_for(m, kT, 1u << 30)), dim3(kT), 0, s, p, m, e);
      };
      scale(cq.p, n4, 10);
      scale(cq.p + n4, 3 * n4, 5);
      scale(cl.p, (size_t)nl * n4, 5);
      scale(x_lo.p, nlo, 5);
      NZ_HIP(hipGetLastError());
    }
  }
  NZ_HIP(hipStreamSynchronize(s));
}

void Prover::init_slots() {
  for (int i = 0; i < kSlots; i++) {
    msc[i].reset(new MsmScratch());
#ifdef NZCB_AB_GENERIC
    msc[i]->init((size_t)n + 6, true, i == 0 ? 3 : 1, true);
#else
    msc[i]->init((size_t)n + 6, true, i == 0 ? 3 : 1, false);
#endif
    NZ_HIP(hipStreamCreateWithFlags(&aux[i], hipStreamNonBlocking));
    NZ_HIP(hipEventCreateWithFlags(&ready[i], hipEventDisableTiming));
  }
  NZ_HIP(hipEventCreateWithFlags(&side_ready, hipEventDisableTiming));
  NZ_HIP(hipEventCreateWithFlags(&side_done, hipEventDisableTiming));
  NZ_HIP(hipEventCreateWithFlags(&pows_done, hipEventDisableTiming));
  mb_apub = kMbEvals + kMbEvalMax;
  mb_pubw = mb_apub + nPublic;
  mb_words = mb_pubw + nPublic;
  NZ_HIP(hipHostMalloc((void**)&top_host, mb_words * sizeof(Fr), hipHostMallocCoherent));
  std::memset((void*)top_host, 0, mb_words * sizeof(Fr));
}

void Prover::alloc_workspace() {
  wit.alloc(nVars ? nVars : 1);
  wtns_in.alloc(nWit ? nWit : 1);
  A.alloc(n + 2); B.alloc(n + 2); C.alloc(n + 2); Z.alloc(n);
  pol_a.alloc(n + 2); pol_b.alloc(n + 2); pol_c.alloc(n + 2); pol_z.alloc(n + 3);
  const size_t ne = quot3 ? (size_t)3 * n : n4;
  A4.alloc(ne); B4.alloc(ne); C4.alloc(ne); Z4.alloc(ne);
  T.alloc(ne); Tz.alloc(ne); t.alloc(quot3 ? ne + 6 : n4);
  pol_r.alloc(n + 3); pol_wxi.alloc(n + 6); pol_wxiw.alloc(n + 3);
  blind.alloc(13);
  scan_tmp.alloc(3 * ((size_t)n / kTileN + 2) + 64);
  lin_qn = (size_t)n / kTileN + 3;
  lin_tab.alloc(2 * sizeof(LinTab) / sizeof(Fr) + 4 * lin_qn);
  lin_host.resize(2 * sizeof(LinTab) / sizeof(Fr));
  size_t nblocks = ((size_t)3 * n + 6 + (size_t)kT * kEvalChunk2 - 1) / ((size_t)kT * kEvalChunk2) + 1;
  eval_part.alloc((size_t)kEvalMax * nblocks + kEvalMax);
  eval_pw.alloc((size_t)kEvalMax * kT + (kEvalMax * kEvalBits * sizeof(Fr) + sizeof(F29) - 1) / sizeof(F29));
  host_part.resize(std::max<size_t>(nblocks, kEvalMax));
  flags.p = (uint32_t*)(blind.p + 12);
  flags.n = 1;
  flags.owned = false;
  const int zlog = quot3 ? power : power + 2;
  if (zlog > 8) ntt_scr2.alloc((size_t)9 << zlog);
}

Prover::Prover(const Prover& pk, int lane) {
  GuardScope guards;
  lane_id = lane;
  n = pk.n; n4 = pk.n4; nVars = pk.nVars; nPublic = pk.nPublic; nAdditions = pk.nAdditions;
  nConstraints = pk.nConstraints; nWit = pk.nWit; power = pk.power;
  k1 = pk.k1; k2 = pk.k2; wn = pk.wn; w2 = pk.w2;
  add_level_start = pk.add_level_start;
  transcript_public = pk.transcript_public;
  for (int k = 0; k < 4; k++) zh_inv[k] = pk.zh_inv[k];
  NZ_HIP(hipSetDevice(pk.eng->device));
  eng.reset(new Engine(pk.eng->device, power + 2, 0));
  init_slots();
  ptau.alias(pk.ptau);
  ptab.q.alias(pk.ptab.q);
  ptab.n = pk.ptab.n; ptab.stride = pk.ptab.stride; ptab.c = pk.ptab.c; ptab.nw = pk.ptab.nw;
  ptab.mont_folded = pk.ptab.mont_folded;
  lcommit = pk.lcommit;
  ltau.alias(pk.ltau);
  ltab.q.alias(pk.ltab.q);
  ltab.n = pk.ltab.n; ltab.stride = pk.ltab.stride; ltab.c = pk.ltab.c; ltab.nw = pk.ltab.nw;
  ltab.sparse = pk.ltab.sparse;
  qm.alias(pk.qm); ql.alias(pk.ql); qr.alias(pk.qr); qo.alias(pk.qo); qc.alias(pk.qc);
  sigma.alias(pk.sigma); sig_h.alias(pk.sig_h); q_h.alias(pk.q_h); w_h.alias(pk.w_h); lagrange.alias(pk.lagrange);
  amap.alias(pk.amap); bmap.alias(pk.bmap); cmap.alias(pk.cmap); adds.alias(pk.adds);
  root_lo.alias(pk.root_lo); root_hi.alias(pk.root_hi); x_lo.alias(pk.x_lo);
  g_lo.alias(pk.g_lo); g_hi.alias(pk.g_hi); gi_lo.alias(pk.gi_lo); gi_hi.alias(pk.gi_hi);
  g29.alias(pk.g29); gi29.alias(pk.gi29);
  cq.alias(pk.cq); cs.alias(pk.cs); cl.alias(pk.cl);
  quot3 = pk.quot3;
  cq3.alias(pk.cq3); cs3.alias(pk.cs3); cl3.alias(pk.cl3);
  tw3.alias(pk.tw3); itw3.alias(pk.itw3);
  for (int j = 0; j < 3; j++) d3[j] = pk.d3[j];
  std::memcpy(sig_top, pk.sig_top, sizeof(sig_top));
  alloc_workspace();
}

void Prover::launch_gate_check(hipStream_t s) {
  hipLaunchKernelGGL(k_gate_h, dim3(grid_for(n, kT, 1u << 30)), dim3(kT), 0, s, A.p, B.p, C.p, q_h.p, (size_t)n,
                     nPublic, flags.p);
  NZ_HIP(hipGetLastError());
}

void Prover::copy_tops(hipStream_t s) {
  hipLaunchKernelGGL(k_tops, dim3(1), dim3(32), 0, s, pol_a.p, pol_b.p, pol_c.p, pol_z.p, (size_t)n,
                     (const uint32_t*)flags.p, top_host);
  NZ_HIP(hipGetLastError());
  NZ_HIP(hipStreamSynchronize(s));
  if (top_host[kMbFlags].v[0] & 1u) throw Error(NZCB_ERR_T_DIV, "T Polynomial is not divisible");
}

void Prover::round3_quot3(const Fr& beta, const Fr& gamma, const Fr& alpha, hipStream_t s) {
  const size_t n3 = (size_t)3 * n;
  const bool side = lcommit;
  if (side) copy_tops(s);
  QArgs29 q29;
  q29.beta = f29_exp(beta, 5);
  q29.k23 = k1 == fr_small(2) && k2 == fr_small(3) ? 1 : 0;
  q29.bk1 = f29_exp(beta * k1, 5);
  q29.bk2 = f29_exp(beta * k2, 5);
  q29.alpha2 = f29_exp(alpha * alpha, 5);
  for (int k = 0; k < 4; k++) q29.zhinv[k] = f29_exp(zh_inv[k], 5);
  q29.gamma = f29_exp(gamma, 0);
  q29.negone = f29_exp(neg(Fr::one()), 0);
  q29.alpha = f29_exp(alpha, 20);
  hipLaunchKernelGGL((k_quotient_coset29<true>), dim3(grid_for(n3, kT, 1u << 30)), dim3(kT), 0, s, A4.p, B4.p, C4.p,
                     Z4.p, cq3.p, cs3.p, cl3.p, nPublic, A.p, (size_t)n, x_lo.p, root_hi.p, q29, T.p);
  if (!side) launch_gate_check(s);
  for (int j = 0; j < 3; j++) {
    NttIo io;
    io.out_f = itw3.p + (size_t)j * n;
    io.out_f_has_scale = true;
    {
      const size_t sp = prof_gpu ? span_begin(1, s) : 0;
      ntt(eng->ntt_tables, T.p + (size_t)j * n, Tz.p + (size_t)j * n, power, true, s, nullptr, &io);
      if (prof_gpu) span_end(sp, s);
    }
  }
  NZ_HIP(hipGetLastError());
  if (!side) copy_tops(s);
  Fr top[4][6];
  std::memcpy(top, top_host, sizeof(top));
  Fr p1[4][6], p2[4][6];
  const Fr w = wn, wi = inverse(wn);
  const Fr wpow[6] = {w * w, w, Fr::one(), wi, wi * wi, wi * wi * wi};
  for (int u = 0; u < 6; u++) {
    for (int f3 = 0; f3 < 3; f3++) {
      p1[f3][u] = top[f3][5 - u];
      p2[f3][u] = top[f3][5 - u];
      if (u >= 2) p2[f3][u] = p2[f3][u] + beta * sig_top[f3][5 - u];
    }
    p1[3][u] = top[3][5 - u];
    p2[3][u] = top[3][5 - u] * wpow[u];
  }
  auto conv = [](const Fr (&x)[6], const Fr (&y)[6], Fr (&out)[6]) {
    for (int s2 = 0; s2 < 6; s2++) {
      Fr acc = Fr::zero();
      for (int u = 0; u <= s2; u++) acc = acc + x[u] * y[s2 - u];
      out[s2] = acc;
    }
  };
  Fr e1[6], e2[6], e3[6], h1[6], h2[6], h3[6];
  conv(p1[0], p1[1], e1);
  conv(e1, p1[2], e2);
  conv(e2, p1[3], e3);
  conv(p2[0], p2[1], h1);
  conv(h1, p2[2], h2);
  conv(h2, p2[3], h3);
  T3Args ta;
  const Fr D = d3[0], D3 = D * D * D, i4 = d3[1] * inverse(D), quarter = inverse(fr_small(4));
  for (int k = 0; k < 6; k++) {
    ta.q3[k] = alpha * (e3[5 - k] - h3[5 - k]);
    const Fr c = D3 * ta.q3[k] * quarter;
    ta.c0[k] = c;
    ta.c1[k] = neg(i4 * c);
    ta.c2[k] = neg(c);
  }
  ta.i4 = i4;
  ta.two_over_d = fr_small(2) * inverse(D);
  ta.inv_d2 = inverse(D * D);
  hipLaunchKernelGGL(k_t_combine, dim3(grid_for(n, kT, 1u << 30)), dim3(kT), 0, s, Tz.p, (size_t)n, ta, t.p);
  NZ_HIP(hipGetLastError());
}

void Prover::to4t(const Fr* evals, Fr* coefs, Fr* evals4, const int* bidx, int nb, hipStream_t s) {
  if (!s) s = st();
  to4t_coefs(evals, coefs, bidx, nb, s);
  to4t_evals4(coefs, evals4, nb, s);
}

void Prover::to4t_coefs(const Fr* evals, Fr* coefs, const int* bidx, int nb, hipStream_t s, uint32_t* scr) {
  auto t0 = std::chrono::steady_clock::now();
  {
    const size_t sp = prof_gpu ? span_begin(1, s) : 0;
    ntt(eng->ntt_tables, evals, coefs, power, true, s, nullptr, nullptr, scr);
    if (prof_gpu) span_end(sp, s);
  }
  BlindIdx bi;
  bi.count = nb;
  for (int k = 0; k < nb; k++) bi.idx[k] = bidx[k];
  hipLaunchKernelGGL(k_blind, dim3(1), dim3(64), 0, s, coefs, (size_t)n, blind.p, bi);
  NZ_HIP(hipGetLastError());
  ntt_ms += ms_since(t0);
}

void Prover::to4t_evals4(const Fr* coefs, Fr* evals4, int nb, hipStream_t s, uint32_t* scr) {
  auto t0 = std::chrono::steady_clock::now();
  if (quot3) {
    for (int j = 0; j < 3; j++) {
      NttIo io;
      io.in_len = n;
      io.in_f = tw3.p + (size_t)j * n;
      io.fold_len = (size_t)nb;
      io.fold_n = n;
      io.fold_f = fr29_operand(d3[j]);
      {
        const size_t sp = prof_gpu ? span_begin(1, s) : 0;
        ntt(eng->ntt_tables, coefs, evals4 + (size_t)j * n, power, false, s, nullptr, &io, scr);
        if (prof_gpu) span_end(sp, s);
      }
    }
    NZ_HIP(hipGetLastError());
    ntt_ms += ms_since(t0);
    return;
  }
  NttIo io;
  io.in_len = (size_t)n + nb;
  io.in_f = g29.p;
  {
    const size_t sp = prof_gpu ? span_begin(1, s) : 0;
    ntt(eng->ntt_tables, coefs, evals4, power + 2, false, s, nullptr, &io, scr);
    if (prof_gpu) span_end(sp, s);
  }
  NZ_HIP(hipGetLastError());
  ntt_ms += ms_since(t0);
}

void Prover::commit_start(int slot, const Fr* coefs, size_t len, const MsmBaseTable* tab, const G1Affine* bases,
                          bool on_main) {
  static const char* const kEnq[kSlots] = {"mark: commit enqueue slot 0", "mark: commit enqueue slot 1",
                                           "mark: commit enqueue slot 2"};
  roctxMarkA(kEnq[slot]);
  NZ_HIP(hipEventRecord(ready[slot], st()));
  hipStream_t ms = on_main ? st() : aux[slot];
  if (!on_main) NZ_HIP(hipStreamWaitEvent(ms, ready[slot], 0));
  const bool lag = tab != nullptr && tab == &ltab;
  slot_lag[slot] = lag;
  slot_split[slot] = false;
  if (!shards.empty() && (!lag || own_lhi)) {
    for (auto& sh : shards) {
      const size_t lo = lag ? sh->llo : sh->lo, hi = lag ? sh->lhi : sh->hi;
      const size_t cnt = len > lo ? std::min(len, hi) - lo : 0;
      NZ_HIP(hipSetDevice(sh->device));
      if (cnt) {
        NZ_HIP(hipStreamWaitEvent(sh->st[slot], ready[slot], 0));
        NZ_HIP(hipMemcpyPeerAsync(sh->scal[slot].p, sh->device, coefs + lo, eng->device, cnt * sizeof(Fr),
                                  sh->st[slot]));
      }
      msm_enqueue(*sh->sc[slot], nullptr, sh->scal[slot].p, cnt, true, sh->st[slot],
                  lag ? &sh->ltable : &sh->table);
    }
    NZ_HIP(hipSetDevice(eng->device));
    len = std::min(len, lag ? own_lhi : own_hi);
    slot_split[slot] = true;
  }
  if (split_send && (!lag || split_own_l)) {
    NZ_HIP(hipEventSynchronize(ready[slot]));
    if (split_send(split_user, slot | (lag ? NZCB_MSM_LAGRANGE : 0), coefs, len) != 0)
      throw Error(NZCB_ERR_INTERNAL, "msm split: sending the scalars to the other ranks failed");
    len = std::min(len, lag ? split_own_l : split_own);
    slot_split[slot] = true;
  }
  const size_t sp = prof_gpu ? span_begin(0, ms) : 0;
  msm_enqueue(*msc[slot], bases ? bases : ptau.p, coefs, len, true, ms, tab ? tab : &ptab);
  if (prof_gpu) span_end(sp, ms);
  static const bool serial = std::getenv("NZCB_SERIAL") != nullptr;
  if (serial) NZ_HIP(hipStreamSynchronize(ms));
  static const char* const kDone[kSlots] = {"mark: commit enqueued slot 0", "mark: commit enqueued slot 1",
                                            "mark: commit enqueued slot 2"};
  roctxMarkA(kDone[slot]);
}

namespace {
void affine_to_le(const G1Affine& a, uint8_t* out) {
  const Fq x = a.is_inf() ? Fq::zero() : from_mont(a.x);
  const Fq y = a.is_inf() ? Fq::zero() : from_mont(a.y);
  std::memcpy(out, x.v, 32);
  std::memcpy(out + 32, y.v, 32);
}

G1xyzz xyzz_from_le(const uint8_t* in) {
  G1Affine a;
  Fq x, y;
  std::memcpy(x.v, in, 32);
  std::memcpy(y.v, in + 32, 32);
  if (x.is_zero() && y.is_zero()) return G1xyzz::inf();
  if (reduce_once(x) != x || reduce_once(y) != y) throw Error(NZCB_ERR_ARG, "msm split: partial not reduced");
  a.x = to_mont(x);
  a.y = to_mont(y);
  return xyzz_from_affine(a);
}
}

G1Affine Prover::commit_finish(int slot) {
  auto t0 = std::chrono::steady_clock::now();
  G1xyzz r = msm_finish(*msc[slot], aux[slot]);
  static const char* const kRes[kSlots] = {"mark: commit result slot 0", "mark: commit result slot 1",
                                           "mark: commit result slot 2"};
  roctxMarkA(kRes[slot]);
  const bool split = slot_split[slot];
  for (auto& sh : shards) {
    if (!split) break;
    NZ_HIP(hipSetDevice(sh->device));
    r = xyzz_add(r, msm_finish(*sh->sc[slot], sh->st[slot]));
  }
  if (!shards.empty()) NZ_HIP(hipSetDevice(eng->device));
  if (split && split_gather) {
    const G1Affine own = xyzz_to_affine(r);
    uint8_t own_le[64];
    affine_to_le(own, own_le);
    std::vector<uint8_t> parts((size_t)split_world * 64);
    if (split_gather(split_user, slot | (slot_lag[slot] ? NZCB_MSM_LAGRANGE : 0), own_le, parts.data()) != 0)
      throw Error(NZCB_ERR_INTERNAL, "msm split: gathering the partial sums failed");
    r = G1xyzz::inf();
    for (int k = 0; k < split_world; k++) r = xyzz_add(r, xyzz_from_le(parts.data() + 64 * (size_t)k));
  }
  msm_ms += ms_since(t0);
  return xyzz_to_affine(r);
}

void Prover::commit_start_abc(size_t len) {
  roctxMarkA("mark: commit enqueue A, B, C");
  const Fr* sc[3] = {A.p, B.p, C.p};
  const size_t sp = prof_gpu ? span_begin(0, st()) : 0;
  msm_enqueue_sets(*msc[0], sc, 3, len, true, st(), &ltab);
  if (prof_gpu) span_end(sp, st());
  roctxMarkA("mark: commit enqueued A, B, C");
}

void Prover::commit_finish_abc(G1Affine& a, G1Affine& b, G1Affine& c) {
  auto t0 = std::chrono::steady_clock::now();
  G1xyzz r[3];
  msm_finish_sets(*msc[0], st(), r);
  roctxMarkA("mark: commit result A, B, C");
  a = xyzz_to_affine(r[0]);
  b = xyzz_to_affine(r[1]);
  c = xyzz_to_affine(r[2]);
  msm_ms += ms_since(t0);
}

void Prover::set_msm_split(int world, size_t own_points, size_t own_lagrange, nzcb_msm_send_fn send,
                           nzcb_msm_gather_fn gather, void* user) {
  if (world <= 1 || !send || !gather) {
    split_send = nullptr;
    split_gather = nullptr;
    split_world = 1;
    split_own = split_own_l = 0;
    return;
  }
  if (!shards.empty()) throw Error(NZCB_ERR_ARG, "msm split: a context splits over devices or over ranks, not both");
  if (own_points == 0 || own_points > ptau.n) throw Error(NZCB_ERR_ARG, "msm split: bad own point count");
  if (own_lagrange > (lcommit ? ltau.n : 0))
    throw Error(NZCB_ERR_ARG, "msm split: bad own Lagrange point count (A, B, C are committed from coefficients "
                              "when the context has no Lagrange basis)");
  split_send = send;
// ... 171 lines not shown
                     amap.p, bmap.p, cmap.p, nConstraints, n, wit.p, nVars, A.p, B.p, C.p, nPublic,
                     top_host + mb_apub, top_host + mb_pubw);
  NZ_HIP(hipGetLastError());
  NZ_HIP(hipStreamSynchronize(s));
  tm[1] = ms_since(T0);

  ranges.next("round1: to4T + commit A, B, C");
  auto t1 = std::chrono::steady_clock::now();
  G1Affine pA, pB, pC, pZ, pT1, pT2, pT3, pWxi, pWxiw;
  {
    const int ba[2] = {2, 1}, bb[2] = {4, 3}, bc[2] = {6, 5};
    const bool abc_sets = lcommit && shards.empty() && !split_send && msc[0]->max_lsets >= 3 && abc_sets_enabled();
    if (lcommit) {
      hipLaunchKernelGGL(k_abc_tail, dim3(1), dim3(64), 0, s, A.p, B.p, C.p, (size_t)n, blind.p);
      NZ_HIP(hipGetLastError());
      NZ_HIP(hipEventRecord(side_ready, s));
      if (abc_sets) {
        lg("multiexp A");
        lg("multiexp B");
        lg("multiexp C");
        commit_start_abc(n + 2);
      } else {
      lg("multiexp A");
      commit_start(0, A.p, n + 2, &ltab, ltau.p);
      lg("multiexp B");
      commit_start(1, B.p, n + 2, &ltab, ltau.p);
      lg("multiexp C");
      }
      hipStream_t ss = aux[2];
      if (!abc_sets) commit_start(2, C.p, n + 2, &ltab, ltau.p, true);
      NZ_HIP(hipStreamWaitEvent(ss, side_ready, 0));
      to4t(A.p, pol_a.p, A4.p, ba, 2, ss);
      to4t(B.p, pol_b.p, B4.p, bb, 2, ss);
      to4t(C.p, pol_c.p, C4.p, bc, 2, ss);
      if (quot3) launch_gate_check(ss);
      NZ_HIP(hipEventRecord(side_done, ss));
    } else {
      to4t(A.p, pol_a.p, A4.p, ba, 2);
      lg("multiexp A");
      commit_start(0, pol_a.p, n + 2);
      to4t(B.p, pol_b.p, B4.p, bb, 2);
      lg("multiexp B");
      commit_start(1, pol_b.p, n + 2);
      to4t(C.p, pol_c.p, C4.p, bc, 2);
      lg("multiexp C");
      commit_start(2, pol_c.p, n + 2);
    }
    if (lcommit && abc_sets) {
      commit_finish_abc(pA, pB, pC);
    } else {
      pA = commit_finish(0);
      pB = commit_finish(1);
      pC = commit_finish(2);
    }
  }
  tm[2] = ms_since(t1);

  ranges.next("round2: grand product Z + commit");
  auto t2 = std::chrono::steady_clock::now();
  Fr beta, gamma;
  const Fr* Apub = top_host + mb_apub;
  {
    std::vector<uint8_t> tr;
    if (transcript_public) {
      for (uint32_t i = 0; i < nPublic; i++) {
        uint8_t be[32];
        fr_to_be(Apub[i], be);
        tr.insert(tr.end(), be, be + 32);
      }
    }
    for (const G1Affine* p : {&pA, &pB, &pC}) {
      uint8_t u[64];
      g1_uncompressed(*p, u);
      tr.insert(tr.end(), u, u + 64);
    }
    beta = hash_to_fr(tr);
    lg("beta: " + fr_dec(beta));
    std::vector<uint8_t> tr2(32);
    fr_to_be(beta, tr2.data());
    gamma = hash_to_fr(tr2);
    lg("gamma: " + fr_dec(gamma));
  }
  {
    PermArgs pa;
    shoup_pair(beta, pa.beta, pa.beta_s);
    shoup_pair(k1 * beta, pa.k1beta, pa.k1beta_s);
    shoup_pair(k2 * beta, pa.k2beta, pa.k2beta_s);
    pa.gamma256 = f29_exp(gamma, 0);
    pa.k23 = k1 == fr_small(2) && k2 == fr_small(3) ? 1 : 0;
    if (fault == NZCB_DEBUG_GENERIC_K) {
      fault = 0;
      pa.k23 = 0;
    }
    const size_t ntiles = (n + kTileN - 1) / kTileN;
    if (ntiles > 1024 * 64) throw Error(NZCB_ERR_INTERNAL, "round 2: domain too large for the tile factors");
    Fr* ntot = scan_tmp.p;
    Fr* dtot = ntot + ntiles;
    Fr* fac = dtot + ntiles;
    Fr* totals = fac + ntiles;
    hipLaunchKernelGGL(k_perm_tile, dim3((unsigned)ntiles), dim3(kT), 0, s, A.p, B.p, C.p, sig_h.p, (size_t)n,
                       w_h.p, pa, Z.p, ntot, dtot);
    hipLaunchKernelGGL(k_perm_factors, dim3(1), dim3(1024), 0, s, (const Fr*)ntot, (const Fr*)dtot, (int)ntiles,
                       fac, top_host + kMbTotals);
    NZ_HIP(hipGetLastError());
    NZ_HIP(hipStreamSynchronize(s));
    const Fr tt[2] = {top_host[kMbTotals], top_host[kMbTotals + 1]};
    if (tt[0] != tt[1]) throw Error(NZCB_ERR_COPY, "Copy constraints does not match");
    hipLaunchKernelGGL(k_apply_tiles, dim3((unsigned)ntiles), dim3(kT), 0, s, Z.p, (size_t)n,
                       (const Fr*)fac, inverse(tt[1]));
    NZ_HIP(hipGetLastError());
    const int bz[3] = {9, 8, 7};
    to4t_coefs(Z.p, pol_z.p, bz, 3, s, ntt_scr2.p);
    lg("multiexp Z");
    commit_start(0, pol_z.p, n + 3);
    to4t_evals4(pol_z.p, Z4.p, 3, s, ntt_scr2.p);
    pZ = commit_finish(0);
  }
  tm[3] = ms_since(t2);

  ranges.next("round3: quotient t + commit T1, T2, T3");
  auto t3 = std::chrono::steady_clock::now();
  Fr alpha;
  {
    std::vector<uint8_t> tr(64);
    g1_uncompressed(pZ, tr.data());
    alpha = hash_to_fr(tr);
    lg("alpha: " + fr_dec(alpha));
  }
  {
    QArgs q;
    q.beta = beta;
    q.gamma = gamma;
    q.alpha = alpha;
    q.alpha2 = alpha * alpha;
    q.bk1 = beta * k1;
    q.bk2 = beta * k2;
    for (int k = 0; k < 4; k++) q.zhinv[k] = zh_inv[k];
    auto tq = std::chrono::steady_clock::now();
    NZ_HIP(hipStreamWaitEvent(s, side_done, 0));
    if (quot3) {
      round3_quot3(beta, gamma, alpha, s);
    } else if (nPublic <= kQ29MaxPub) {
      QArgs29 q29;
      q29.beta = f29_exp(beta, 5);
      q29.k23 = k1 == fr_small(2) && k2 == fr_small(3) ? 1 : 0;
      q29.bk1 = f29_exp(q.bk1, 5);
      q29.bk2 = f29_exp(q.bk2, 5);
      q29.alpha2 = f29_exp(q.alpha2, 5);
      for (int k = 0; k < 4; k++) q29.zhinv[k] = f29_exp(zh_inv[k], 5);
      q29.gamma = f29_exp(gamma, 0);
      q29.negone = f29_exp(neg(Fr::one()), 0);
      q29.alpha = f29_exp(alpha, 20);
      hipLaunchKernelGGL((k_quotient_coset29<false>), dim3(grid_for(n4, kT, 1u << 30)), dim3(kT), 0, s, A4.p, B4.p,
                         C4.p, Z4.p, cq.p, cs.p, cl.p, nPublic, A.p, (size_t)n, x_lo.p, root_hi.p, q29, T.p);
    } else {
      hipLaunchKernelGGL(k_quotient_coset, dim3(grid_for(n4, kT, 1u << 30)), dim3(kT), 0, s, A4.p, B4.p, C4.p,
                         Z4.p, cq.p, cs.p, cl.p, nPublic, A.p, (size_t)n, x_lo.p, root_hi.p, q, T.p);
    }
    NZ_HIP(hipGetLastError());
    if (!quot3) {
      NttIo io;
      io.out_f = gi29.p;
      io.out_f_has_scale = true;
      io.out_limit = (size_t)3 * n + 6;
      io.out_flags = flags.p;
      {
        const size_t sp = prof_gpu ? span_begin(1, s) : 0;
        ntt(eng->ntt_tables, T.p, t.p, power + 2, true, s, nullptr, &io);
        if (prof_gpu) span_end(sp, s);
      }
      NZ_HIP(hipGetLastError());
      uint32_t f = 0;
      NZ_HIP(hipMemcpyAsync(&f, flags.p, 4, hipMemcpyDeviceToHost, s));
      NZ_HIP(hipStreamSynchronize(s));
      if (f & 1u) throw Error(NZCB_ERR_T_DIV, "T Polynomial is not divisible");
    }
    ntt_ms += ms_since(tq);
    if (fault == NZCB_FAULT_QUOTIENT) {
      fault = 0;
      hipLaunchKernelGGL(k_fault_bump, dim3(1), dim3(64), 0, s, t.p + 1);
      NZ_HIP(hipGetLastError());
    }
    lg("multiexp T1");
    commit_start(0, t.p, n);
    lg("multiexp T2");
    commit_start(1, t.p + n, n);
    lg("multiexp T3");
    commit_start(2, t.p + 2 * (size_t)n, n + 6);
    pT1 = commit_finish(0);
    pT2 = commit_finish(1);
    pT3 = commit_finish(2);
  }
  tm[4] = ms_since(t3);

  ranges.next("round4: evaluations");
  auto t4 = std::chrono::steady_clock::now();
  Fr xi, ea, eb, ec, es1, es2, et, ezw, er, xim;
  {
    std::vector<uint8_t> tr(192);
    g1_uncompressed(pT1, tr.data());
    g1_uncompressed(pT2, tr.data() + 64);
    g1_uncompressed(pT3, tr.data() + 128);
    xi = hash_to_fr(tr);
    lg("xi: " + fr_dec(xi));
    {
      const Fr* polys[7] = {pol_a.p, pol_b.p, pol_c.p, sigma.p, sigma.p + 5 * (size_t)n, t.p, pol_z.p};
      const size_t lens[7] = {n + 2, n + 2, n + 2, n, n, 3 * (size_t)n + 6, n + 3};
      const Fr xs[7] = {xi, xi, xi, xi, xi, xi, xi * wn};
      Fr ev[7];
      eval_many(7, polys, lens, xs, ev, [&] {
        lin_tables(0, xi, aux[2]);
        lin_tables(1, xi * wn, aux[2]);
        NZ_HIP(hipEventRecord(pows_done, aux[2]));
      });
      NZ_HIP(hipStreamWaitEvent(s, pows_done, 0));
      ea = ev[0];
      eb = ev[1];
      ec = ev[2];
      es1 = ev[3];
      es2 = ev[4];
      et = ev[5];
      ezw = ev[6];
    }
    Fr coef_ab = ea * eb;
    Fr betaxi = beta * xi;
    Fr e2 = (ea + betaxi + gamma) * (eb + betaxi * k1 + gamma);
    e2 = e2 * (ec + betaxi * k2 + gamma) * alpha;
    Fr e3 = (ea + beta * es1 + gamma) * (eb + beta * es2 + gamma);
    e3 = e3 * beta * ezw * alpha;
    xim = xi;
    for (int i = 0; i < power; i++) xim = sqr(xim);
    Fr eval_l1 = (xim - Fr::one()) * inverse((xi - Fr::one()) * fr_small(n));
    Fr e4 = eval_l1 * (alpha * alpha);
    RArgs ra{e2 + e4, coef_ab, ea, eb, ec, e3};
    hipLaunchKernelGGL(k_pol_r, dim3(grid_for(n + 3, kT, 1u << 30)), dim3(kT), 0, s, pol_z.p, qm.p, ql.p, qr.p,
                       qo.p, qc.p, sigma.p + 10 * (size_t)n, (size_t)n, ra, pol_r.p);
    NZ_HIP(hipGetLastError());
    {
      const Fr* polys[1] = {pol_r.p};
      const size_t lens[1] = {n + 3};
      eval_many(1, polys, lens, &xi, &er);
    }
    {
      const Fr zh = xim - Fr::one(), nf = fr_small(n);
      Fr pi = Fr::zero(), wj = Fr::one();
      for (uint32_t j = 0; j < nPublic; j++) {
        pi = pi - Apub[j] * wj * zh * inverse(nf * (xi - wj));
        wj = wj * wn;
      }
      const Fr perm = alpha * (ea + beta * es1 + gamma) * (eb + beta * es2 + gamma) * (ec + gamma) * ezw;
      if (et * zh != er + pi - perm - e4)
        throw Error(NZCB_ERR_INTERNAL, "quotient check failed: t(xi) Z_H(xi) differs from the numerator at xi");
    }
  }
  tm[5] = ms_since(t4);

  ranges.next("round5: Wxi, Wxiw + commit");
  auto t5 = std::chrono::steady_clock::now();
  {
    std::vector<uint8_t> tr(7 * 32);
    const Fr* ev[7] = {&ea, &eb, &ec, &es1, &es2, &ezw, &er};
    for (int i = 0; i < 7; i++) fr_to_be(*ev[i], tr.data() + 32 * i);
    WArgs wa;
    wa.v[0] = Fr::zero();
    wa.v[1] = hash_to_fr(tr);
    lg("v: " + fr_dec(wa.v[1]));
    for (int i = 2; i <= 6; i++) wa.v[i] = wa.v[i - 1] * wa.v[1];
    wa.xim = xim;
    wa.xi2m = xim * xim;
    wa.w0sub = et + wa.v[1] * er + wa.v[2] * ea + wa.v[3] * eb + wa.v[4] * ec + wa.v[5] * es1 + wa.v[6] * es2;
    hipLaunchKernelGGL(k_pol_wxi, dim3(grid_for(n + 6, kT, 1u << 30)), dim3(kT), 0, s, t.p, pol_r.p, pol_a.p,
                       pol_b.p, pol_c.p, sigma.p, sigma.p + 5 * (size_t)n, (size_t)n, wa, T.p);
    NZ_HIP(hipGetLastError());
    div_pol1(T.p, n + 6, 0, Fr::zero(), pol_wxi.p, 4u);
    lg("multiexp Wxi");
    commit_start(0, pol_wxi.p, n + 6);
    div_pol1(pol_z.p, n + 3, 1, ezw, pol_wxiw.p, 4u);
    lg("multiexp Wxiw");
    commit_start(1, pol_wxiw.p, n + 3);
    NZ_HIP(hipStreamSynchronize(s));
    const uint32_t f = top_host[kMbFlags].v[0];
    pWxi = commit_finish(0);
    pWxiw = commit_finish(1);
    if (f & 4u) throw Error(NZCB_ERR_DIVPOL, "Polinomial does not divide");
  }
  tm[6] = ms_since(t5);
  tm[0] = ms_since(T0);
  tm[7] = msm_ms;
  tm[8] = ntt_ms;
  tm[9] = tm[10] = -1;
  if (prof_gpu) span_totals(&tm[9], &tm[10]);

  const G1Affine* pts[9] = {&pA, &pB, &pC, &pZ, &pT1, &pT2, &pT3, &pWxi, &pWxiw};
  for (int i = 0; i < 9; i++) {
    uint8_t* o = proof_out + 64 * i;
    if (pts[i]->is_inf()) {
      std::memset(o, 0, 64);
    } else {
      Fq x = from_mont(pts[i]->x), y = from_mont(pts[i]->y);
      std::memcpy(o, x.v, 32);
      std::memcpy(o + 32, y.v, 32);
    }
  }
  const Fr* ev[7] = {&ea, &eb, &ec, &es1, &es2, &ezw, &er};
  for (int i = 0; i < 7; i++) fr_to_le_normal(*ev[i], proof_out + 9 * 64 + 32 * i);
  for (uint32_t i = 0; i < nPublic; i++) {
    fr_to_le_normal(top_host[mb_pubw + i], pub_out + 32 * (size_t)i);
// ... 5 lines not shown
```

nzcb-circom_amd/nzcb/__init__.py:

```python
from __future__ import annotations

import ctypes
import json
import os
from ctypes import POINTER, c_char, c_double, c_int, c_size_t, c_uint8, c_uint32, c_uint64, c_void_p

_HERE = os.path.dirname(os.path.abspath(__file__))
LIB_PATH = os.environ.get("NZCB_LIB", os.path.join(os.path.dirname(_HERE), "lib", "libnzcb.so"))

PROOF_BYTES = 9 * 64 + 7 * 32
BLINDING_BYTES = 11 * 32
VK_BYTES = 8 + 2 * 32 + 8 * 64 + 4 * 32 + 32
PROOF_POINTS = ("A", "B", "C", "Z", "T1", "T2", "T3", "Wxi", "Wxiw")
PROOF_EVALS = ("eval_a", "eval_b", "eval_c", "eval_s1", "eval_s2", "eval_zw", "eval_r")
VK_POINTS = ("Qm", "Ql", "Qr", "Qo", "Qc", "S1", "S2", "S3")

ERROR_NAMES = {
    0: "OK", 1: "ARG", 2: "FORMAT", 3: "NOT_PLONK", 4: "CURVE", 5: "WITNESS_LEN", 6: "COPY",
    7: "T_DIV", 8: "TZ", 9: "DIVPOL", 10: "HIP", 11: "INTERNAL",
}

EXPORTED_SYMBOLS = [
    "nzcb_version", "nzcb_device_count", "nzcb_ctx_create", "nzcb_ctx_destroy", "nzcb_ctx_set_logger",
    "nzcb_ctx_set_transcript_public", "nzcb_ctx_info", "nzcb_prove", "nzcb_prove_witness", "nzcb_prove_device",
    "nzcb_ctx_kernel_stats",
    "nzcb_ctx_last_timings", "nzcb_proof_to_json", "nzcb_public_to_json", "nzcb_synth_setup", "nzcb_free",
    "nzcb_engine_create", "nzcb_engine_destroy", "nzcb_engine_ntt", "nzcb_engine_msm", "nzcb_dev_alloc",
    "nzcb_dev_free", "nzcb_memcpy_h2d", "nzcb_memcpy_d2h", "nzcb_engine_ntt_dev", "nzcb_engine_msm_dev",
    "nzcb_engine_time_ntt", "nzcb_engine_fr_mul", "nzcb_engine_random_fr", "nzcb_engine_fixed_base",
    "nzcb_engine_time_msm", "nzcb_engine_msm_fixed_dev", "nzcb_engine_msm_table_dev", "nzcb_engine_msm_sets_dev", "nzcb_engine_time_msm2", "nzcb_ctx_set_lanes",
    "nzcb_ctx_lanes", "nzcb_prove_batch", "nzcb_vk_from_zkey", "nzcb_vk_from_zkey_file", "nzcb_vk_to_json", "nzcb_verify",
    "nzcb_proof_to_calldata", "nzcb_vk_to_solidity", "nzcb_engine_lagrange_basis", "nzcb_ctx_set_msm_devices", "nzcb_nzcp_input_signals", "nzcb_nzcp_witness",
    "nzcb_nzcp_witness_dev", "nzcb_synth_setup_ex", "nzcb_memcpy_d2d",
    "nzcb_plonk_setup", "nzcb_prove_batch_status", "nzcb_wprog_remap", "nzcb_prove_logged", "nzcb_memcpy_d2d_async",
    "nzcb_debug_guard_check", "nzcb_debug_guard_selftest", "nzcb_debug_inject_fault", "nzcb_debug_f29",
    "nzcb_msm_table_create_lagrange",
    "nzcb_verify_batch", "nzcb_engine_g1_lincomb", "nzcb_engine_verify_batch", "nzcb_debug_verify_batch_timings",
    "nzcb_r1cs_create", "nzcb_r1cs_create_file", "nzcb_r1cs_info", "nzcb_r1cs_check", "nzcb_r1cs_destroy",
    "nzcb_engine_r1cs_create", "nzcb_debug_r1cs_check_timings",
    "nzcb_p256_key_create", "nzcb_p256_verify", "nzcb_p256_key_destroy", "nzcb_engine_p256_key_create",
    "nzcb_debug_p256_field", "nzcb_debug_p256_mul2", "nzcb_debug_p256_timings",
    "nzcb_nzcp_pass_layout", "nzcb_nzcp_decode", "nzcb_nzcp_decode_dev", "nzcb_debug_nzcp_decode_timings",
]

NZCB_FAULT_QUOTIENT = 1
NZCB_DEBUG_GENERIC_K = 2
NZCB_FAULT_LANE_ALLOC = 3
VERIFY_HOST = -1
R1CS_HOST = -1
WITNESS_WTNS, WITNESS_HOST, WITNESS_DEVICE = 0, 1, 2
P256_HOST = -1
SIG_OK, SIG_INVALID, SIG_RANGE = 0, 1, 2
NZCP_HOST = -1
PASS_MAX_URI = 2048
PASS_STATUS_NAMES = ("OK", "LENGTH", "PREFIX", "BASE32", "TRUNCATED", "CBOR", "NOT_COSE", "HEADER",
                     "CLAIMS")
PASS_HAS_ALG, PASS_HAS_KID, PASS_HAS_ISS, PASS_HAS_NBF, PASS_HAS_EXP, PASS_HAS_CTI, PASS_HAS_SIG = (
    1, 2, 4, 8, 16, 32, 64)
P256_OPS = {"add": 0, "sub": 1, "mul": 2, "sqr": 3, "inv": 4}


def lagrange_commit_enabled() -> bool:
    import re
    e = os.environ.get("NZCB_LAGRANGE_COMMIT")
    if e is None:
        return True
    m = re.match(r"\s*[+-]?\d+", e)
    return bool(m) and int(m.group()) != 0


def guard_check(device: int = -1) -> int:
    err, checked, bad = _Err(), c_size_t(0), c_int(0)
    _check(load().nzcb_debug_guard_check(device, ctypes.byref(checked), ctypes.byref(bad), ctypes.byref(err)), err)
    return checked.value


F29_WORDS = {1: (27, 9), 2: (54, 18), 3: (18, 9), 4: (36, 18), 5: (18, 18), 6: (36, 9)}


def f29_check(op: int, words, device: int = 0):
    win, wout = F29_WORDS[op]
    count = len(words) // win
    assert count * win == len(words)
    arr = (c_uint32 * max(1, len(words)))(*words)
    out = (c_uint32 * max(1, count * wout))()
    err = _Err()
    _check(load().nzcb_debug_f29(device, op, arr, count, out, ctypes.byref(err)), err)
    return list(out)[:count * wout]


def guard_selftest(device: int = 0) -> None:
    err = _Err()
    _check(load().nzcb_debug_guard_selftest(device, ctypes.byref(err)), err)


class NzcbError(RuntimeError):
    def __init__(self, code: int, msg: str):
        super().__init__(msg)
        self.code = code
        self.name = ERROR_NAMES.get(code, str(code))


class _Err(ctypes.Structure):
    _fields_ = [("code", c_int), ("msg", c_char * 256)]


class NzcpParams(ctypes.Structure):
    _fields_ = [("is_live", ctypes.c_int32), ("max_tbs_bytes", ctypes.c_int32),
                ("max_array_len_vc", ctypes.c_int32), ("max_map_len_vc", ctypes.c_int32)]


class NzcpRecord(ctypes.Structure):
    _fields_ = [("status", ctypes.c_int32), ("detail", ctypes.c_int32), ("exp", ctypes.c_uint32),
                ("vc_pos", ctypes.c_int32), ("given_len", ctypes.c_int32), ("family_len", ctypes.c_int32),
                ("dob_len", ctypes.c_int32), ("nullifier_len", ctypes.c_int32),
                ("tbs_sha256", c_uint8 * 32), ("nullifier_sha512", c_uint8 * 64), ("nullifier", c_uint8 * 64),
                ("pub", (c_uint8 * 32) * 3)]


class NzcpPass(ctypes.Structure):
    _fields_ = [("status", ctypes.c_int32), ("detail", c_uint32), ("version", c_uint32), ("present", c_uint32),
                ("alg", ctypes.c_int32), ("kid_len", c_uint32), ("iss_len", c_uint32), ("cti_len", c_uint32),
                ("sig_len", c_uint32), ("cose_len", c_uint32), ("protected_off", c_uint32),
                ("protected_len", c_uint32), ("payload_off", c_uint32), ("payload_len", c_uint32),
                ("tbs_len", c_uint32), ("fits", c_uint32), ("nbf", c_uint64), ("exp", c_uint64),
                ("kid", c_uint8 * 32), ("cti", c_uint8 * 32), ("iss", c_uint8 * 64), ("sig", c_uint8 * 64),
                ("tbs_sha256", c_uint8 * 32)]


NZCP_LIVE = dict(is_live=1, max_tbs_bytes=351, max_array_len_vc=0, max_map_len_vc=4)
NZCP_EXAMPLE = dict(is_live=0, max_tbs_bytes=314, max_array_len_vc=0, max_map_len_vc=4)

LOG_FN = ctypes.CFUNCTYPE(None, c_void_p, ctypes.c_char_p)
MSM_SEND_FN = ctypes.CFUNCTYPE(c_int, c_void_p, c_int, c_void_p, c_size_t)
MSM_GATHER_FN = ctypes.CFUNCTYPE(c_int, c_void_p, c_int, POINTER(c_uint8), POINTER(c_uint8))
MSM_LAGRANGE = 0x100

_lib = None


def load(path: str | None = None):
    global _lib
    if _lib is not None and path is None:
        return _lib
    if os.environ.get("GPU_MAX_HW_QUEUES", "4") == "4":
        os.environ["GPU_MAX_HW_QUEUES"] = "24"
    lib = ctypes.CDLL(path or LIB_PATH)
    u8p = POINTER(c_uint8)
    sigs = {
        "nzcb_version": (ctypes.c_char_p, []),
        "nzcb_device_count": (c_int, []),
        "nzcb_ctx_create": (c_void_p, [u8p, c_size_t, c_int, POINTER(_Err)]),
        "nzcb_ctx_destroy": (None, [c_void_p]),
        "nzcb_ctx_set_logger": (None, [c_void_p, LOG_FN, c_void_p]),
        "nzcb_ctx_set_transcript_public": (None, [c_void_p, c_int]),
        "nzcb_ctx_info": (c_int, [c_void_p, POINTER(c_uint32)]),
        "nzcb_prove": (c_int, [c_void_p, u8p, c_size_t, u8p, u8p, u8p, c_size_t, POINTER(_Err)]),
        "nzcb_prove_witness": (c_int, [c_void_p, u8p, c_size_t, u8p, u8p, u8p, c_size_t, POINTER(_Err)]),
        "nzcb_prove_device": (c_int, [c_void_p, c_void_p, c_size_t, u8p, u8p, u8p, c_size_t, POINTER(_Err)]),
        "nzcb_prove_logged": (c_int, [c_void_p, c_void_p, c_size_t, c_int, u8p, u8p, u8p, c_size_t, LOG_FN, c_void_p,
                                      POINTER(_Err)]),
        "nzcb_ctx_kernel_stats": (c_int, [c_void_p, c_int, POINTER(c_double)]),
        "nzcb_ctx_set_lanes": (c_int, [c_void_p, c_int, POINTER(_Err)]),
        "nzcb_ctx_set_msm_devices": (c_int, [c_void_p, POINTER(c_int), c_int, POINTER(_Err)]),
        "nzcb_vk_from_zkey": (c_int, [u8p, c_size_t, u8p, POINTER(_Err)]),
        "nzcb_vk_from_zkey_file": (c_int, [ctypes.c_char_p, u8p, POINTER(_Err)]),
        "nzcb_vk_to_json": (c_int, [u8p, ctypes.c_char_p, c_size_t]),
        "nzcb_verify": (c_int, [u8p, u8p, u8p, c_int, c_int, POINTER(c_int), POINTER(_Err)]),
        "nzcb_proof_to_calldata": (c_int, [u8p, u8p, c_int, ctypes.c_char_p, c_size_t]),
        "nzcb_vk_to_solidity": (c_int, [u8p, ctypes.c_char_p, c_int, ctypes.c_char_p, c_size_t]),
        "nzcb_engine_lagrange_basis": (c_int, [c_void_p, c_void_p, c_size_t, c_int, c_void_p, POINTER(_Err)]),
        "nzcb_ctx_lanes": (c_int, [c_void_p]),
        "nzcb_prove_batch": (c_int, [c_void_p, POINTER(c_void_p), c_size_t, c_int, c_int, u8p, u8p, u8p, c_size_t,
                                     POINTER(_Err)]),
        "nzcb_prove_batch_status": (c_int, [c_void_p, POINTER(c_void_p), c_size_t, c_int, c_int, u8p, u8p, u8p,
                                            c_size_t, POINTER(c_int), POINTER(_Err)]),
        "nzcb_ctx_last_timings": (c_int, [c_void_p, POINTER(c_double), c_int]),
        "nzcb_proof_to_json": (c_int, [u8p, ctypes.c_char_p, c_size_t]),
        "nzcb_public_to_json": (c_int, [u8p, c_int, ctypes.c_char_p, c_size_t]),
        "nzcb_synth_setup": (c_int, [c_int, c_int, c_int, c_uint64, c_uint32, u8p, c_int,
                                     POINTER(POINTER(c_uint8)), POINTER(c_size_t),
                                     POINTER(POINTER(c_uint8)), POINTER(c_size_t), POINTER(_Err)]),
        "nzcb_synth_setup_ex": (c_int, [c_int, c_int, c_int, c_uint64, c_uint32, c_uint32, u8p, c_int,
                                        POINTER(POINTER(c_uint8)), POINTER(c_size_t),
                                        POINTER(POINTER(c_uint8)), POINTER(c_size_t), POINTER(_Err)]),
        "nzcb_free": (None, [c_void_p]),
        "nzcb_engine_create": (c_void_p, [c_int, c_int, c_size_t, POINTER(_Err)]),
        "nzcb_engine_destroy": (None, [c_void_p]),
        "nzcb_engine_ntt": (c_int, [c_void_p, u8p, u8p, c_int, c_int, POINTER(_Err)]),
        "nzcb_engine_msm": (c_int, [c_void_p, u8p, u8p, c_size_t, c_int, u8p, POINTER(_Err)]),
        "nzcb_dev_alloc": (c_void_p, [c_size_t]),
        "nzcb_dev_alloc_on": (c_void_p, [c_int, c_size_t]),
        "nzcb_dev_free": (None, [c_void_p]),
        "nzcb_memcpy_h2d": (c_int, [c_void_p, c_void_p, c_size_t]),
        "nzcb_memcpy_d2h": (c_int, [c_void_p, c_void_p, c_size_t]),
        "nzcb_memcpy_d2d": (c_int, [c_void_p, c_void_p, c_size_t]),
        "nzcb_memcpy_d2d_async": (c_int, [c_void_p, c_void_p, c_size_t, c_void_p]),
        "nzcb_engine_ntt_dev": (c_int, [c_void_p, c_void_p, c_void_p, c_int, c_int, POINTER(_Err)]),
        "nzcb_engine_msm_dev": (c_int, [c_void_p, c_void_p, c_void_p, c_size_t, c_int, u8p, POINTER(_Err)]),
        "nzcb_engine_time_ntt": (c_int, [c_void_p, c_void_p, c_void_p, c_int, c_int, c_int, POINTER(c_double),
                                         POINTER(_Err)]),
        "nzcb_engine_fr_mul": (c_int, [c_void_p, u8p, u8p, u8p, c_size_t, c_int, POINTER(_Err)]),
        "nzcb_engine_random_fr": (c_int, [c_void_p, c_void_p, c_size_t, c_uint64, POINTER(_Err)]),
        "nzcb_engine_fixed_base": (c_int, [c_void_p, c_void_p, c_size_t, c_void_p, POINTER(_Err)]),
        "nzcb_engine_time_msm": (c_int, [c_void_p, c_void_p, c_void_p, c_size_t, c_int, c_int, POINTER(c_double),
                                         POINTER(c_double), POINTER(_Err)]),
        "nzcb_engine_msm_fixed_dev": (c_int, [c_void_p, c_void_p, c_size_t, c_void_p, c_size_t, c_int, u8p,
                                              POINTER(_Err)]),
        "nzcb_engine_msm_table_dev": (c_int, [c_void_p, c_void_p, c_size_t, c_void_p, c_size_t, c_int, c_int, c_int,
                                              c_int, u8p, POINTER(_Err)]),
        "nzcb_engine_msm_sets_dev": (c_int, [c_void_p, c_void_p, c_size_t, POINTER(c_void_p), c_int, c_size_t, c_int,
                                             c_int, u8p, POINTER(_Err)]),
        "nzcb_plonk_setup": (c_int, [ctypes.c_char_p, c_size_t, ctypes.c_char_p, c_size_t, c_int, POINTER(POINTER(c_uint8)),
                                     POINTER(c_size_t), POINTER(_Err)]),
        "nzcb_nzcp_input_signals": (c_size_t, [POINTER(NzcpParams)]),
        "nzcb_nzcp_witness": (c_int, [c_int, POINTER(NzcpParams), u8p, c_int, POINTER(NzcpRecord), POINTER(_Err)]),
        "nzcb_nzcp_witness_dev": (c_int, [c_int, POINTER(NzcpParams), c_void_p, c_int, c_void_p, c_void_p, c_size_t,
                                          c_void_p, POINTER(_Err)]),
        "nzcb_engine_time_msm2": (c_int, [c_void_p, c_void_p, c_void_p, c_size_t, c_int, c_int, c_int,
                                          POINTER(c_double), POINTER(_Err)]),
        "nzcb_ctx_create_devices": (c_void_p, [u8p, c_size_t, POINTER(c_int), c_int, POINTER(_Err)]),
        "nzcb_ctx_devices": (c_int, [c_void_p]),
        "nzcb_ctx_set_msm_split": (c_int, [c_void_p, c_int, c_size_t, c_size_t, MSM_SEND_FN, MSM_GATHER_FN,
                                           c_void_p, POINTER(_Err)]),
        "nzcb_msm_table_create": (c_void_p, [c_int, c_void_p, c_size_t, POINTER(_Err)]),
        "nzcb_msm_table_create_lagrange": (c_void_p, [c_int, c_void_p, c_size_t, c_int, c_size_t, c_size_t,
                                                      POINTER(_Err)]),
        "nzcb_msm_table_run": (c_int, [c_void_p, c_void_p, c_size_t, c_int, u8p, POINTER(_Err)]),
        "nzcb_msm_table_destroy": (None, [c_void_p]),
        "nzcb_ptau_synth": (c_int, [c_int, u8p, c_int, POINTER(POINTER(c_uint8)), POINTER(c_size_t), POINTER(_Err)]),
        "nzcb_wprog_create": (c_void_p, [ctypes.c_char_p, c_size_t, c_int, POINTER(_Err)]),
        "nzcb_wprog_destroy": (None, [c_void_p]),
        "nzcb_wprog_info": (c_int, [c_void_p, POINTER(c_uint32)]),
        "nzcb_wprog_run_dev": (c_int, [c_void_p, c_void_p, c_int, c_void_p, c_size_t, POINTER(ctypes.c_int32),
                                       c_void_p, POINTER(_Err)]),
        "nzcb_wprog_run": (c_int, [c_void_p, ctypes.c_char_p, c_int, u8p, POINTER(ctypes.c_int32), POINTER(_Err)]),
        "nzcb_wprog_remap": (c_int, [ctypes.c_char_p, c_size_t, ctypes.c_char_p, c_size_t, ctypes.c_char_p, c_size_t,
                                     POINTER(POINTER(c_uint8)), POINTER(c_size_t), POINTER(c_uint32), POINTER(_Err)]),
        "nzcb_debug_guard_check": (c_int, [c_int, POINTER(c_size_t), POINTER(c_int), POINTER(_Err)]),
        "nzcb_debug_guard_selftest": (c_int, [c_int, POINTER(_Err)]),
        "nzcb_debug_inject_fault": (c_int, [c_void_p, c_int]),
        "nzcb_debug_f29": (c_int, [c_int, c_int, POINTER(c_uint32), c_size_t, POINTER(c_uint32), POINTER(_Err)]),
        "nzcb_verify_batch": (c_int, [u8p, u8p, u8p, c_size_t, c_int, c_int, c_int, c_int, u8p, POINTER(c_int),
                                      POINTER(_Err)]),
        "nzcb_engine_g1_lincomb": (c_int, [c_int, u8p, u8p, POINTER(c_uint32), c_size_t, u8p, POINTER(_Err)]),
        "nzcb_engine_verify_batch": (c_int, [u8p, u8p, u8p, c_size_t, c_int, c_int, c_int, c_int, u8p, POINTER(c_int),
                                             u8p, POINTER(c_int), POINTER(_Err)]),
        "nzcb_debug_verify_batch_timings": (c_int, [POINTER(c_double), c_int]),
        "nzcb_r1cs_create": (c_void_p, [ctypes.c_char_p, c_size_t, c_int, POINTER(_Err)]),
        "nzcb_r1cs_create_file": (c_void_p, [ctypes.c_char_p, c_int, POINTER(_Err)]),
        "nzcb_engine_r1cs_create": (c_void_p, [ctypes.c_char_p, c_size_t, c_int, c_uint32, c_int, POINTER(_Err)]),
        "nzcb_r1cs_info": (c_int, [c_void_p, POINTER(c_uint32)]),
        "nzcb_r1cs_check": (c_int, [c_void_p, c_void_p, c_size_t, c_int, c_int, c_size_t, POINTER(c_uint32),
                                    POINTER(c_uint32), c_uint32, c_void_p, POINTER(_Err)]),
        "nzcb_r1cs_destroy": (None, [c_void_p]),
        "nzcb_debug_r1cs_check_timings": (c_int, [POINTER(c_double), c_int]),
        "nzcb_p256_key_create": (c_void_p, [ctypes.c_char_p, c_int, POINTER(_Err)]),
        "nzcb_engine_p256_key_create": (c_void_p, [ctypes.c_char_p, c_int, c_int, POINTER(_Err)]),
        "nzcb_p256_verify": (c_int, [c_void_p, c_void_p, c_size_t, c_void_p, c_size_t, c_int, c_int,
                                     POINTER(ctypes.c_int32), c_void_p, POINTER(_Err)]),
        "nzcb_p256_key_destroy": (None, [c_void_p]),
        "nzcb_debug_p256_field": (c_int, [c_int, c_int, c_int, ctypes.c_char_p, ctypes.c_char_p, c_size_t, u8p,
                                          POINTER(_Err)]),
        "nzcb_debug_p256_mul2": (c_int, [c_void_p, ctypes.c_char_p, ctypes.c_char_p, c_size_t, u8p, POINTER(_Err)]),
        "nzcb_debug_p256_timings": (c_int, [POINTER(c_double), c_int]),
        "nzcb_nzcp_pass_layout": (None, [POINTER(c_uint32)]),
        "nzcb_nzcp_decode": (c_int, [c_int, ctypes.c_char_p, POINTER(c_uint32), c_int, POINTER(NzcpParams),
                                     ctypes.c_char_p, POINTER(NzcpPass), u8p, u8p, c_size_t, POINTER(_Err)]),
        "nzcb_nzcp_decode_dev": (c_int, [c_int, c_void_p, c_void_p, c_int, POINTER(NzcpParams), c_void_p, c_void_p,
                                         c_void_p, c_void_p, c_size_t, c_void_p, POINTER(_Err)]),
        "nzcb_debug_nzcp_decode_timings": (c_int, [POINTER(c_double), c_int]),
    }
    lib.missing_symbols = []
    for name, (res, args) in sigs.items():
        try:
            fn = getattr(lib, name)
        except AttributeError:
            lib.missing_symbols.append(name)
            continue
        fn.restype = res
        fn.argtypes = args
    if "nzcb_nzcp_pass_layout" not in lib.missing_symbols:
        lay = (c_uint32 * 3)()
        lib.nzcb_nzcp_pass_layout(lay)
        if list(lay) != [ctypes.sizeof(NzcpPass), NzcpPass.sig.offset, NzcpPass.tbs_sha256.offset]:
            raise OSError(f"NzcpPass does not mirror nzcb_nzcp_pass: the library reports {list(lay)}")
    _lib = lib
    return lib


def _buf(data: bytes):
    return (c_uint8 * len(data)).from_buffer_copy(data) if data else (c_uint8 * 1)()


def _out(n: int):
    return (c_uint8 * max(n, 1))()


def _check(rc: int, err: _Err):
    if rc != 0:
        raise NzcbError(rc, err.msg.decode(errors="replace"))


def version() -> str:
    return load().nzcb_version().decode()


def device_count() -> int:
    return load().nzcb_device_count()


def nzcp_input_signals(params: dict) -> int:
    return load().nzcb_nzcp_input_signals(ctypes.byref(NzcpParams(**params)))


def _record_dict(r: NzcpRecord) -> dict:
    return {
        "status": r.status, "detail": r.detail, "exp": r.exp, "vc_pos": r.vc_pos, "given_len": r.given_len,
        "family_len": r.family_len, "dob_len": r.dob_len, "nullifier_len": r.nullifier_len,
        "tbs_sha256": bytes(r.tbs_sha256), "nullifier_sha512": bytes(r.nullifier_sha512),
        "nullifier": bytes(r.nullifier), "out": [int.from_bytes(bytes(r.pub[k]), "little") for k in range(3)],
    }


def nzcp_witness(inputs: bytes, count: int, params: dict = NZCP_LIVE, device: int = 0) -> list:
    lib = load()
    prm = NzcpParams(**params)
    need = lib.nzcb_nzcp_input_signals(ctypes.byref(prm)) * 32 * count
    if len(inputs) != need:
        raise ValueError(f"nzcp inputs are {len(inputs)} bytes, expected {need}")
    recs = (NzcpRecord * max(count, 1))()
    err = _Err()
    _check(lib.nzcb_nzcp_witness(device, ctypes.byref(prm), _buf(inputs), count, recs, ctypes.byref(err)), err)
    return [_record_dict(recs[i]) for i in range(count)]


def nzcp_witness_dev(dev_inputs: int, count: int, params: dict = NZCP_LIVE, device: int = 0,
                     dev_records: int | None = None, dev_witness: int | None = None, witness_stride: int = 0,
                     stream: int | None = None):
    lib = load()
    err = _Err()
    _check(lib.nzcb_nzcp_witness_dev(device, ctypes.byref(NzcpParams(**params)), dev_inputs, count, dev_records,
                                     dev_witness, witness_stride, stream, ctypes.byref(err)), err)


def nzcp_records_from_bytes(raw: bytes, count: int) -> list:
    size = ctypes.sizeof(NzcpRecord)
    return [_record_dict(NzcpRecord.from_buffer_copy(raw[i * size:(i + 1) * size])) for i in range(count)]


def _pass_dict(r: NzcpPass) -> dict:
    has = lambda bit: bool(r.present & bit)
    return {
        "status": r.status, "status_name": PASS_STATUS_NAMES[r.status], "detail": r.detail, "version": r.version,
        "present": r.present, "alg": r.alg if has(PASS_HAS_ALG) else None,
        "kid": bytes(r.kid)[:min(r.kid_len, 32)] if has(PASS_HAS_KID) else None, "kid_len": r.kid_len,
        "iss": bytes(r.iss)[:min(r.iss_len, 64)].decode(errors="replace") if has(PASS_HAS_ISS) else None,
        "iss_len": r.iss_len, "nbf": r.nbf if has(PASS_HAS_NBF) else None,
        "exp": r.exp if has(PASS_HAS_EXP) else None,
        "cti": bytes(r.cti)[:min(r.cti_len, 32)] if has(PASS_HAS_CTI) else None, "cti_len": r.cti_len,
        "sig": bytes(r.sig) if has(PASS_HAS_SIG) else None, "sig_len": r.sig_len, "cose_len": r.cose_len,
        "protected_off": r.protected_off, "protected_len": r.protected_len, "payload_off": r.payload_off,
        "payload_len": r.payload_len, "tbs_len": r.tbs_len, "fits": r.fits, "tbs_sha256": bytes(r.tbs_sha256),
    }


def nzcp_passes_from_bytes(raw: bytes, count: int) -> list:
    size = ctypes.sizeof(NzcpPass)
    return [_pass_dict(NzcpPass.from_buffer_copy(raw[i * size:(i + 1) * size])) for i in range(count)]


def pack_uris(uris):
    raw = [u.encode("utf-8", "surrogateescape") if isinstance(u, str) else bytes(u) for u in uris]
    offs, at = [0], 0
    for b in raw:
        at += len(b)
        offs.append(at)
    if at > 1 << 31:
        raise ValueError("more than 2^31 bytes of URIs")
    return b"".join(raw), (c_uint32 * len(offs))(*offs)


def nzcp_decode_raw(uris, params: dict | None = None, data20=None, device: int = 0, want_tbs: int = 0,
                    offsets=None):
    lib = load()
    if offsets is None:
        blob, offs = pack_uris(uris)
    else:
        blob, offs = bytes(uris), (c_uint32 * len(offsets))(*offsets)
    count = len(offs) - 1
    if data20 is not None:
        data20 = b"".join(data20) if isinstance(data20, (list, tuple)) else bytes(data20)
        if len(data20) != 20 * count:
            raise ValueError("data is 20 bytes per pass")
    prm = NzcpParams(**params) if params else None
    recs = (NzcpPass * max(count, 1))()
    inputs = _out(lib.nzcb_nzcp_input_signals(ctypes.byref(prm)) * 32 * count) if prm else None
    tbs = _out(want_tbs * count) if want_tbs else None
    err = _Err()
    _check(lib.nzcb_nzcp_decode(device, blob, offs, count, ctypes.byref(prm) if prm else None, data20, recs, inputs,
                                tbs, want_tbs, ctypes.byref(err)), err)
    size = ctypes.sizeof(NzcpPass)
    return (bytes(recs)[:size * count],
            bytes(inputs)[:lib.nzcb_nzcp_input_signals(ctypes.byref(prm)) * 32 * count] if prm else None,
            bytes(tbs)[:want_tbs * count] if want_tbs else None)


def nzcp_decode(uris, params: dict | None = None, data20=None, device: int = 0):
    uris = list(uris)
    recs, inputs, _ = nzcp_decode_raw(uris, params, data20, device)
    out = nzcp_passes_from_bytes(recs, len(uris))
    return (out, inputs) if params else out


def nzcp_decode_dev(dev_uris: int, dev_offsets: int, count: int, dev_passes: int, params: dict | None = None,
                    dev_data20: int | None = None, dev_inputs: int | None = None, dev_tbs: int | None = None,
                    tbs_stride: int = 0, device: int = 0, stream: int | None = None):
    lib = load()
    err = _Err()
    prm = NzcpParams(**params) if params else None
    _check(lib.nzcb_nzcp_decode_dev(device, dev_uris, dev_offsets, count, ctypes.byref(prm) if prm else None,
                                    dev_data20, dev_passes, dev_inputs, dev_tbs, tbs_stride, stream,
                                    ctypes.byref(err)), err)


def nzcp_decode_timings() -> list:
    ms = (c_double * 2)()
    n = load().nzcb_debug_nzcp_decode_timings(ms, 2)
    return list(ms)[:n]


class Engine:

    def __init__(self, device: int = 0, max_log_ntt: int = 12, max_msm_points: int = 1 << 12):
        self.lib = load()
        err = _Err()
        self.h = self.lib.nzcb_engine_create(device, max_log_ntt, max_msm_points, ctypes.byref(err))
        if not self.h:
            raise NzcbError(err.code, err.msg.decode(errors="replace"))

    def close(self):
        if self.h:
            self.lib.nzcb_engine_destroy(self.h)
            self.h = None

    __del__ = close

    def ntt(self, data_lem: bytes, log_n: int, inverse: bool = False) -> bytes:
        n = 1 << log_n
        assert len(data_lem) == 32 * n
        out = _out(32 * n)
        err = _Err()
        _check(self.lib.nzcb_engine_ntt(self.h, _buf(data_lem), out, log_n, int(inverse), ctypes.byref(err)), err)
        return bytes(out)

    def msm(self, bases_lem: bytes, scalars: bytes, scalars_mont: bool = False) -> bytes:
        n = len(scalars) // 32
        assert len(bases_lem) == 64 * n
        out = _out(64)
        err = _Err()
        _check(self.lib.nzcb_engine_msm(self.h, _buf(bases_lem), _buf(scalars), n, int(scalars_mont), out,
                                        ctypes.byref(err)), err)
        return bytes(out)

    def field_mul(self, a_lem: bytes, b_lem: bytes, field_q: bool = False) -> bytes:
        n = len(a_lem) // 32
        out = _out(32 * n)
        err = _Err()
        _check(self.lib.nzcb_engine_fr_mul(self.h, _buf(a_lem), _buf(b_lem), out, n, int(field_q),
                                           ctypes.byref(err)), err)
        return bytes(out)

    def time_ntt(self, dev_in: int, dev_out: int, log_n: int, inverse: bool, reps: int) -> float:
        ms = c_double()
        err = _Err()
        _check(self.lib.nzcb_engine_time_ntt(self.h, dev_in, dev_out, log_n, int(inverse), reps, ctypes.byref(ms),
                                             ctypes.byref(err)), err)
        return ms.value

    def random_fr(self, dev_out: int, n: int, seed: int):
        err = _Err()
        _check(self.lib.nzcb_engine_random_fr(self.h, dev_out, n, seed, ctypes.byref(err)), err)

    def fixed_base(self, dev_scalars: int, n: int, dev_out: int):
        err = _Err()
        _check(self.lib.nzcb_engine_fixed_base(self.h, dev_scalars, n, dev_out, ctypes.byref(err)), err)

    def lagrange_basis(self, dev_ptau: int, ptau_n: int, log_n: int, dev_out: int):
        err = _Err()
        _check(self.lib.nzcb_engine_lagrange_basis(self.h, dev_ptau, ptau_n, log_n, dev_out, ctypes.byref(err)), err)

    def time_msm(self, dev_bases: int, dev_scalars: int, n: int, scalars_mont: bool, reps: int):
        ms = c_double()
        acc = c_double()
        err = _Err()
        _check(self.lib.nzcb_engine_time_msm(self.h, dev_bases, dev_scalars, n, int(scalars_mont), reps,
                                             ctypes.byref(ms), ctypes.byref(acc), ctypes.byref(err)), err)
        return ms.value, acc.value

    MSM_PHASES = ("keys", "sort", "offsets", "accumulate", "finalize", "reduce", "sums")

    def time_msm_phases(self, dev_bases: int, dev_scalars: int, n: int, scalars_mont: bool, fixed_base: bool,
                        reps: int) -> dict:
        out = (c_double * 13)()
        err = _Err()
        _check(self.lib.nzcb_engine_time_msm2(self.h, dev_bases, dev_scalars, n, int(scalars_mont), int(fixed_base),
                                              reps, out, ctypes.byref(err)), err)
        d = {"wall": out[0], "table_build": out[8], "entries": out[9]}
        d.update({k: out[1 + i] for i, k in enumerate(self.MSM_PHASES)})
        d["host_finish"] = out[10]
        d["host_enqueue"] = out[11]
        d["host_sort_call"] = out[12]
        return d

    def msm_fixed_dev(self, dev_bases: int, n_table: int, dev_scalars: int, n: int, scalars_mont: bool,
                      window: int = 0, sparse: bool = False, fold: bool = False) -> bytes:
        out = _out(64)
        err = _Err()
        if window or sparse or fold:
            _check(self.lib.nzcb_engine_msm_table_dev(self.h, dev_bases, n_table, dev_scalars, n, int(scalars_mont),
                                                      int(window), int(sparse), int(fold), out, ctypes.byref(err)),
                   err)
        else:
            _check(self.lib.nzcb_engine_msm_fixed_dev(self.h, dev_bases, n_table, dev_scalars, n, int(scalars_mont),
                                                      out, ctypes.byref(err)), err)
        return bytes(out)

    def msm_sets_dev(self, dev_bases: int, n_table: int, dev_scalars: list, n: int, scalars_mont: bool, *,
                     sparse: bool) -> list:
        k = len(dev_scalars)
        out = _out(64 * k)
        err = _Err()
        arr = (c_void_p * k)(*dev_scalars)
        _check(self.lib.nzcb_engine_msm_sets_dev(self.h, dev_bases, n_table, arr, k, n, int(scalars_mont),
                                                 int(bool(sparse)), out, ctypes.byref(err)), err)
        return [bytes(out)[64 * i:64 * i + 64] for i in range(k)]

    def msm_dev(self, dev_bases: int, dev_scalars: int, n: int, scalars_mont: bool) -> bytes:
        out = _out(64)
        err = _Err()
        _check(self.lib.nzcb_engine_msm_dev(self.h, dev_bases, dev_scalars, n, int(scalars_mont), out,
                                            ctypes.byref(err)), err)
        return bytes(out)

    @staticmethod
    def g1_lincomb(points: bytes, scalars: bytes, group_end, device: int = 0) -> list:
        groups = len(group_end)
        n = group_end[-1] if groups else 0
        assert len(points) == 64 * n and len(scalars) == 32 * n
        ends = (c_uint32 * max(groups, 1))(*group_end)
        out = _out(64 * groups)
        err = _Err()
        _check(load().nzcb_engine_g1_lincomb(device, _buf(points), _buf(scalars), ends, groups, out,
                                             ctypes.byref(err)), err)
        return [bytes(out)[64 * g:64 * g + 64] for g in range(groups)]

    @staticmethod
    def verify_batch(vk: bytes, proofs, publics, transcript_public: bool = True, device: int = 0,
                     seed: bytes | None = None, n_public: int | None = None):
        count = len(proofs)
        assert len(publics) == count and all(len(p) == PROOF_BYTES for p in proofs)
        if n_public is None:
            n_public = len(publics[0]) // 32 if count else 0
        stride = max([32 * n_public] + [len(p) for p in publics])
        pubs = b"".join(bytes(p).ljust(stride, b"\0") for p in publics)
        assert seed is None or len(seed) == 32
        valid = (c_int * max(count, 1))()
        pts = _out(128 * count)
        checks = c_int(0)
        err = _Err()
        _check(load().nzcb_engine_verify_batch(_buf(vk), _buf(b"".join(proofs)), _buf(pubs), stride, n_public, count,
                                               int(transcript_public), device, _buf(seed) if seed else None, valid,
                                               pts, ctypes.byref(checks), ctypes.byref(err)), err)
        raw = bytes(pts)
        return ([bool(valid[i]) for i in range(count)], [raw[128 * i:128 * i + 128] for i in range(count)],
                checks.value)

    @staticmethod
    def verify_batch_timings() -> list:
        ms = (c_double * 6)()
        k = load().nzcb_debug_verify_batch_timings(ms, 6)
        return list(ms)[:k]


def dev_alloc(nbytes: int) -> int:
    p = load().nzcb_dev_alloc(nbytes)
    if not p:
        raise NzcbError(10, "hipMalloc failed")
    return p


def dev_free(p: int):
    load().nzcb_dev_free(p)


def h2d(dst: int, data: bytes):
    buf = ctypes.create_string_buffer(data, len(data))
    rc = load().nzcb_memcpy_h2d(dst, buf, len(data))
    if rc:
        raise NzcbError(rc, "h2d failed")


def memcpy_h2d_ptr(dst: int, src_addr: int, nbytes: int):
    rc = load().nzcb_memcpy_h2d(dst, src_addr, nbytes)
    if rc:
        raise NzcbError(rc, "h2d failed")


# ... 878 lines not shown
```

Before: 47.16 proofs/s.

## Fold coset shift into NTT twiddles and simplify quotient scaling

Replaces the per-element coset pre-multiplication (in_f table of n factors) in the 3-coset quotient NTTs with precomputed coset-twisted twiddle tables. The first stage now also uses twiddles, and each stage's factors are absorbed into its table. Inverse-NTT 1/n scaling becomes a shift-by-2^k Montgomery division instead of a full multiply. The first unit-twiddle radix-4 stage is specialised, beta*x_lo is precomputed once per proof, and the zh_inv multiply moves from the quotient kernel into the inverse coset factors. Risks include correctness of the new twiddle layout and extra table memory; a debug coset-NTT entry point is added for testing.

```diff
diff --git a/include/nzcb_internal.h b/include/nzcb_internal.h
--- a/include/nzcb_internal.h
+++ b/include/nzcb_internal.h
@@ -32,6 +32,8 @@
 int nzcb_engine_ntt(nzcb_engine* e, const uint8_t* in_lem, uint8_t* out_lem, int log_n, int inverse, nzcb_err* err);
 int nzcb_engine_msm(nzcb_engine* e, const uint8_t* bases_lem, const uint8_t* scalars, size_t n, int scalars_mont,
                     uint8_t* out_affine, nzcb_err* err);
+int nzcb_debug_ntt_coset(nzcb_engine* e, const uint8_t* in_lem, uint8_t* out_lem, int log_n, const uint8_t* c_lem,
+                         int fold_len, nzcb_err* err);
 int nzcb_engine_ntt_dev(nzcb_engine* e, const void* in, void* out, int log_n, int inverse, nzcb_err* err);
 int nzcb_engine_msm_dev(nzcb_engine* e, const void* bases, const void* scalars, size_t n, int scalars_mont,
                         uint8_t* out_affine, nzcb_err* err);
diff --git a/nzcb-circom_amd/csrc/capi_engine.hip b/nzcb-circom_amd/csrc/capi_engine.hip
--- a/nzcb-circom_amd/csrc/capi_engine.hip
+++ b/nzcb-circom_amd/csrc/capi_engine.hip
@@ -214,6 +214,37 @@
   DevBuf<Fr> a(n), b(n);
   NZ_HIP(hipMemcpyAsync(a.p, in_lem, n * 32, hipMemcpyHostToDevice, g.stream));
   ntt(g.ntt_tables, a.p, b.p, log_n, inverse != 0, g.stream);
+  NZ_HIP(hipMemcpyAsync(out_lem, b.p, n * 32, hipMemcpyDeviceToHost, g.stream));
+  NZ_HIP(hipStreamSynchronize(g.stream));
+  return 0;
+  NZ_GUARD_END(err)
+}
+
+int nzcb_debug_ntt_coset(nzcb_engine* e, const uint8_t* in_lem, uint8_t* out_lem, int log_n, const uint8_t* c_lem,
+                         int fold_len, nzcb_err* err) {
+  NZ_GUARD_BEGIN
+  Engine& g = e->eng;
+  if (log_n < 1 || log_n > g.ntt_tables.max_log || fold_len < 0 || (size_t)fold_len > (size_t(1) << log_n))
+    throw Error(NZCB_ERR_ARG, "ntt coset: 1 <= log_n <= the engine's, 0 <= fold_len <= n");
+  NZ_HIP(hipSetDevice(g.device));
+  const size_t n = size_t(1) << log_n;
+  Fr c;
+  std::memcpy(c.v, c_lem, 32);
+  DevBuf<Fr> a(n + (size_t)fold_len), b(n);
+  DevBuf<NttTables::Tw> tw(n - 1);
+  NZ_HIP(hipMemcpyAsync(a.p, in_lem, (n + (size_t)fold_len) * 32, hipMemcpyHostToDevice, g.stream));
+  ntt_coset_twiddles(g.ntt_tables, c, log_n, tw.p, g.stream);
+  NttIo io;
+  io.in_len = n;
+  io.tw = tw.p;
+  if (fold_len) {
+    Fr d = pow_u64(c, (uint64_t)n);
+    for (int k = 0; k < 5; k++) d = d + d;
+    io.fold_len = (size_t)fold_len;
+    io.fold_n = n;
+    io.fold_f = split29(d);
+  }
+  ntt(g.ntt_tables, a.p, b.p, log_n, false, g.stream, nullptr, &io);
   NZ_HIP(hipMemcpyAsync(out_lem, b.p, n * 32, hipMemcpyDeviceToHost, g.stream));
   NZ_HIP(hipStreamSynchronize(g.stream));
   return 0;
diff --git a/nzcb-circom_amd/csrc/f29.h b/nzcb-circom_amd/csrc/f29.h
--- a/nzcb-circom_amd/csrc/f29.h
+++ b/nzcb-circom_amd/csrc/f29.h
@@ -583,6 +583,28 @@
   return join_fr29(r);
 }
 
+NZ_HD F29 div2k29(const F29& x, int K) {
+  using Q = Fr29;
+  const uint32_t m = (x.v[0] * Q::INV) & ((1u << K) - 1u);
+  uint32_t t[8];
+  uint64_t acc = 0;
+#pragma unroll
+  for (int l = 0; l < 8; l++) {
+    acc += x.v[l];
+    mad29c(acc, m, Q::P[l]);
+    t[l] = (uint32_t)acc & Q::MASK;
+    acc >>= 29;
+  }
+  acc += x.v[8];
+  mad29c(acc, m, Q::P[8]);
+  F29 r;
+#pragma unroll
+  for (int l = 0; l < 7; l++) r.v[l] = (t[l] >> K) | ((t[l + 1] << (29 - K)) & Q::MASK);
+  r.v[7] = (t[7] >> K) | ((uint32_t)(acc << (29 - K)) & Q::MASK);
+  r.v[8] = (uint32_t)(acc >> K);
+  return r;
+}
+
 NZ_HD F29 fr_to261(const Fr& x) {
   const F29 r = split29(x);
   F29 o;
diff --git a/nzcb-circom_amd/csrc/f29_check.hip b/nzcb-circom_amd/csrc/f29_check.hip
--- a/nzcb-circom_amd/csrc/f29_check.hip
+++ b/nzcb-circom_amd/csrc/f29_check.hip
@@ -5,8 +5,8 @@
 namespace nzcb {
 namespace {
 
-constexpr int kIn[7] = {0, 27, 54, 18, 36, 18, 36};
-constexpr int kOut[7] = {0, 9, 18, 9, 18, 18, 9};
+constexpr int kIn[8] = {0, 27, 54, 18, 36, 18, 36, 10};
+constexpr int kOut[8] = {0, 9, 18, 9, 18, 18, 9, 9};
 
 __device__ __forceinline__ F29 ld(const uint32_t* p) {
   F29 r;
@@ -45,8 +45,11 @@
     sqr29x2(ld(a), ld(a + 9), r1, r2);
     st(o, r1);
     st(o + 9, r2);
+  } else if constexpr (OP == 6) {
+    st(o, mul2sum29(ld(a), ld(a + 9), ld(a + 18), ld(a + 27)));
   } else {
-    st(o, mul2sum29(ld(a), ld(a + 9), ld(a + 18), ld(a + 27)));
+    const uint32_t k = a[9];
+    st(o, div2k29(ld(a), (int)(k < 1 ? 1 : k > 28 ? 28 : k)));
   }
 }
 
@@ -68,8 +71,8 @@
     }
     return code;
   };
-  if (op < 1 || op > 6 || (count && (!in || !out)) || count > (size_t(1) << 24))
-    return fail(NZCB_ERR_ARG, "f29 check: op 1..6, count <= 2^24");
+  if (op < 1 || op > 7 || (count && (!in || !out)) || count > (size_t(1) << 24))
+    return fail(NZCB_ERR_ARG, "f29 check: op 1..7, count <= 2^24");
   try {
     if (count) {
       NZ_HIP(hipSetDevice(device));
@@ -81,7 +84,8 @@
         case 3: launch<3>(din.p, dout.p, count); break;
         case 4: launch<4>(din.p, dout.p, count); break;
         case 5: launch<5>(din.p, dout.p, count); break;
-        default: launch<6>(din.p, dout.p, count); break;
+        case 6: launch<6>(din.p, dout.p, count); break;
+        default: launch<7>(din.p, dout.p, count); break;
       }
       NZ_HIP(hipGetLastError());
       NZ_HIP(hipMemcpy(out, dout.p, count * kOut[op] * 4, hipMemcpyDeviceToHost));
diff --git a/nzcb-circom_amd/csrc/ntt.h b/nzcb-circom_amd/csrc/ntt.h
--- a/nzcb-circom_amd/csrc/ntt.h
+++ b/nzcb-circom_amd/csrc/ntt.h
@@ -25,7 +25,10 @@
   bool out_f_has_scale = false;
   size_t out_limit = ~size_t(0);
   uint32_t* out_flags = nullptr;
+  const NttTables::Tw* tw = nullptr;
 };
+
+void ntt_coset_twiddles(const NttTables& t, const Fr& c, int log_n, NttTables::Tw* out, hipStream_t st);
 
 void ntt(const NttTables& t, const Fr* in, Fr* out, int log_n, bool inverse, hipStream_t st,
          const Fr* scale = nullptr, const NttIo* io = nullptr, uint32_t* scratch29 = nullptr);
diff --git a/nzcb-circom_amd/csrc/ntt.hip b/nzcb-circom_amd/csrc/ntt.hip
--- a/nzcb-circom_amd/csrc/ntt.hip
+++ b/nzcb-circom_amd/csrc/ntt.hip
@@ -36,17 +36,48 @@
   out[i] = full[k << (L - g - 1)];
 }
 
+__device__ __forceinline__ NttTables::Tw tw29_of(const Fr& s) {
+  Fr m = s;
+#pragma unroll
+  for (int k = 0; k < 5; k++) m = m + m;
+  NttTables::Tw t;
+  t.w = split29(from_mont(s));
+  t.ws = mul_lo261(split29(m), f29_const(Fr29::NINV));
+  return t;
+}
 __global__ void __launch_bounds__(256) ntt_tw29_kernel(NttTables::Tw* __restrict__ out, const Fr* __restrict__ tw,
                                                        size_t count) {
   size_t i = (size_t)blockIdx.x * blockDim.x + threadIdx.x;
   if (i >= count) return;
-  Fr m = tw[i];
-#pragma unroll
-  for (int k = 0; k < 5; k++) m = m + m;
-  NttTables::Tw t;
-  t.w = split29(from_mont(tw[i]));
-  t.ws = mul_lo261(split29(m), f29_const(Fr29::NINV));
-  out[i] = t;
+  out[i] = tw29_of(tw[i]);
+}
+
+struct CosetStageF {
+  F29 f[28];
+};
+__global__ void __launch_bounds__(256)
+ntt_coset_tw29_kernel(NttTables::Tw* __restrict__ out, const NttTables::Tw* __restrict__ plain, CosetStageF cf,
+                      size_t count) {
+  size_t i = (size_t)blockIdx.x * blockDim.x + threadIdx.x;
+  if (i >= count) return;
+  const int g = 63 - __clzll((unsigned long long)(i + 1));
+  out[i] = tw29_of(join_fr29(mul29<Fr29>(plain[i].w, cf.f[g])));
+}
+
+void ntt_coset_twiddles(const NttTables& t, const Fr& c, int L, NttTables::Tw* out, hipStream_t st) {
+  if (L < 1 || L > t.max_log || L > 28) throw Error(NZCB_ERR_ARG, "ntt coset twiddles: size exceeds table");
+  CosetStageF cf = {};
+  Fr f = c;
+  for (int g = L - 1; g >= 0; g--) {
+    Fr op = to_mont(f);
+    for (int k = 0; k < 5; k++) op = op + op;
+    cf.f[g] = split29(op);
+    f = sqr(f);
+  }
+  const size_t total = (size_t(1) << L) - 1;
+  hipLaunchKernelGGL(ntt_coset_tw29_kernel, dim3(grid_for(total, 256, 1u << 30)), dim3(256), 0, st, out,
+                     (const NttTables::Tw*)t.fwd29.p, cf, total);
+  NZ_HIP(hipGetLastError());
 }
 
 void NttTables::init(int L, hipStream_t st) {
@@ -116,6 +147,47 @@
   for (int l = 0; l < 9; l++) r.v[l] = a.v[l] + Fr29::K4[l] - b.v[l];
   return r;
 }
+__device__ __forceinline__ F29 sub8r_nn29(const F29& a, const F29& b) {
+  F29 r;
+#pragma unroll
+  for (int l = 0; l < 9; l++) r.v[l] = a.v[l] + 2u * Fr29::K4[l] - b.v[l];
+  return r;
+}
+
+template <bool UNIT>
+__device__ __forceinline__ void radix4_group(uint32_t* sl, int i0, int i1, int i2, int i3,
+                                             const NttTables::Tw* __restrict__ wa, const NttTables::Tw* __restrict__ wb,
+                                             const NttTables::Tw* __restrict__ wc) {
+  F29 t1 = tile_ld(sl, i1), t3 = tile_ld(sl, i3);
+  if (!UNIT) {
+    const NttTables::Tw w = *wa;
+    F29 p1, p3;
+    tw_mul2(t1, w, t3, w, p1, p3);
+    t1 = p1;
+    t3 = p3;
+  }
+  const F29 x0 = tile_ld(sl, i0), x2 = tile_ld(sl, i2);
+  const F29 y0 = add_nn29(x0, t1), y1 = sub4r_nn29(x0, t1);
+  const F29 y2 = add_nn29(x2, t3), y3 = sub4r_nn29(x2, t3);
+  F29 u2, u3, z2;
+  if (!UNIT) {
+    tw_mul2(y2, *wb, y3, *wc, u2, u3);
+    z2 = sub4r_nn29(y0, u2);
+  } else {
+    u2 = y2;
+    u3 = tw_mul(y3, *wc);
+    z2 = sub8r_nn29(y0, y2);
+  }
+  F29 z0 = add_nn29(y0, u2), z1 = add_nn29(y1, u3), z3 = sub4r_nn29(y1, u3);
+  norm29(z0);
+  norm29(z1);
+  norm29(z2);
+  norm29(z3);
+  tile_st(sl, i0, z0);
+  tile_st(sl, i1, z1);
+  tile_st(sl, i2, z2);
+  tile_st(sl, i3, z3);
+}
 
 template <bool IN29, bool OUT29>
 __global__ void __launch_bounds__(kTile / 4)
@@ -149,7 +221,8 @@
           }
         }
         if (io.in_f) x = mul29<Fr29>(x, io.in_f[src]);
-        if (do_scale) x = mul29<Fr29>(x, scale29);
+        if (do_scale == 2) x = div2k29(x, L);
+        else if (do_scale) x = mul29<Fr29>(x, scale29);
       }
       tile_st(sl, e, x);
     }
@@ -165,7 +238,9 @@
   }
   __syncthreads();
   const int nbf = n_el >> 1;
+  const int ngroups = n_el >> 2;
   const bool first = !IN29;
+  const bool twist = !IN29 && io.tw != nullptr;
   int st = 0;
   if (sparse4 && blockIdx.x != 0) {
     for (int e = tid; e < n_el; e += T) {
@@ -187,7 +262,7 @@
       const size_t k = first ? 0 : (lo0 + c);
       const F29 x0 = tile_ld(sl, i0);
       const F29 x1 = tile_ld(sl, i1);
-      const F29 tt = g ? tw_mul(x1, twg[k]) : x1;
+      const F29 tt = (g || twist) ? tw_mul(x1, twg[k]) : x1;
       F29 y0 = add_nn29(x0, tt), y1 = sub4r_nn29(x0, tt);
       norm29(y0);
       norm29(y1);
@@ -196,8 +271,17 @@
     }
     __syncthreads();
     st = 1;
-  }
-  const int ngroups = n_el >> 2;
+  } else if (!IN29 && !twist && q >= 2) {
+    const int b = tid;
+    if (b < ngroups) {
+      const int c = b & (C - 1);
+      const int j = (b >> logC) << 2;
+      radix4_group<true>(sl, (j << logC) + c, ((j + 1) << logC) + c, ((j + 2) << logC) + c, ((j + 3) << logC) + c,
+                         tw, tw, tw + 2);
+    }
+    __syncthreads();
+    st = 2;
+  }
 #pragma unroll 1
   for (; st < q; st += 2) {
     const int h = 1 << st;
@@ -212,31 +296,8 @@
       const int j = ((pr >> st) << (st + 2)) | low;
       const size_t ka = first ? (size_t)low : (((size_t)low << s) + lo0 + c);
       const size_t kc = first ? (size_t)(low + h) : (((size_t)(low + h) << s) + lo0 + c);
-      const int i0 = (j << logC) + c, i1 = ((j + h) << logC) + c, i2 = ((j + 2 * h) << logC) + c,
-                i3 = ((j + 3 * h) << logC) + c;
-      F29 t1 = tile_ld(sl, i1), t3 = tile_ld(sl, i3);
-      if (g) {
-        const NttTables::Tw wa = twa[ka];
-        F29 p1, p3;
-        tw_mul2(t1, wa, t3, wa, p1, p3);
-        t1 = p1;
-        t3 = p3;
-      }
-      const F29 x0 = tile_ld(sl, i0), x2 = tile_ld(sl, i2);
-      const F29 y0 = add_nn29(x0, t1), y1 = sub4r_nn29(x0, t1);
-      const F29 y2 = add_nn29(x2, t3), y3 = sub4r_nn29(x2, t3);
-      F29 u2, u3;
-      const NttTables::Tw wb = twb[ka], wc = twb[kc];
-      tw_mul2(y2, wb, y3, wc, u2, u3);
-      F29 z0 = add_nn29(y0, u2), z2 = sub4r_nn29(y0, u2), z1 = add_nn29(y1, u3), z3 = sub4r_nn29(y1, u3);
-      norm29(z0);
-      norm29(z1);
-      norm29(z2);
-      norm29(z3);
-      tile_st(sl, i0, z0);
-      tile_st(sl, i1, z1);
-      tile_st(sl, i2, z2);
-      tile_st(sl, i3, z3);
+      radix4_group<false>(sl, (j << logC) + c, ((j + h) << logC) + c, ((j + 2 * h) << logC) + c,
+                          ((j + 3 * h) << logC) + c, twa + ka, twb + ka, twb + kc);
     }
     __syncthreads();
   }
@@ -306,13 +367,18 @@
   if (in == out) throw Error(NZCB_ERR_ARG, "ntt requires in != out");
   F29* scr = (F29*)(scratch29 ? scratch29 : t.scratch29.p);
   if (L > 8 && !scratch29 && t.scratch29.n < ((size_t)9 << L)) throw Error(NZCB_ERR_INTERNAL, "ntt: no scratch");
-  const NttTables::Tw* tw = inverse_dir ? t.inv29.p : t.fwd29.p;
+  if (io.tw && inverse_dir) throw Error(NZCB_ERR_ARG, "ntt: coset twiddles are for the forward transform");
+  const NttTables::Tw* tw = io.tw ? io.tw : inverse_dir ? t.inv29.p : t.fwd29.p;
   Fr sc = Fr::one();
   int do_scale = 0;
   if (inverse_dir && !io.out_f_has_scale) {
-    Fr two = Fr::one() + Fr::one();
-    sc = inverse(pow_u64(two, (uint64_t)L));
-    do_scale = 1;
+    if (!scale && L >= 1 && L <= 28) {
+      do_scale = 2;
+    } else {
+      Fr two = Fr::one() + Fr::one();
+      sc = inverse(pow_u64(two, (uint64_t)L));
+      do_scale = 1;
+    }
   }
   if (scale) {
     sc = do_scale ? sc * *scale : *scale;
diff --git a/nzcb-circom_amd/csrc/prover.h b/nzcb-circom_amd/csrc/prover.h
--- a/nzcb-circom_amd/csrc/prover.h
+++ b/nzcb-circom_amd/csrc/prover.h
@@ -65,7 +65,8 @@
   DevBuf<Fr> cq, cs, cl;
   bool quot3 = false;
   DevBuf<Fr> cq3, cs3, cl3;
-  DevBuf<F29> tw3, itw3;
+  DevBuf<NttTables::Tw> ctw3;
+  DevBuf<F29> itw3;
   Fr d3[3];
   Fr sig_top[3][4];
   DevBuf<Fr> wit;
@@ -73,6 +74,7 @@
   DevBuf<Fr> A, B, C, Z;
   DevBuf<Fr> pol_a, pol_b, pol_c, pol_z;
   DevBuf<Fr> A4, B4, C4, Z4, T, Tz, t;
+  DevBuf<Fr> bx_lo;
   DevBuf<Fr> pol_r, pol_wxi, pol_wxiw;
   DevBuf<Fr> blind;
   DevBuf<Fr> scan_tmp;
diff --git a/nzcb-circom_amd/csrc/prover.hip b/nzcb-circom_amd/csrc/prover.hip
--- a/nzcb-circom_amd/csrc/prover.hip
+++ b/nzcb-circom_amd/csrc/prover.hip
@@ -550,7 +550,8 @@
 k_quotient_coset29(const Fr* __restrict__ A, const Fr* __restrict__ B, const Fr* __restrict__ C,
                    const Fr* __restrict__ Z, const Fr* __restrict__ cq, const Fr* __restrict__ cs,
                    const Fr* __restrict__ cl, uint32_t npub, const Fr* __restrict__ Apub, size_t n,
-                   const Fr* __restrict__ xlo, const Fr* __restrict__ xhi, QArgs29 q, Fr* __restrict__ T) {
+                   const Fr* __restrict__ xlo, const Fr* __restrict__ xhi, const Fr* __restrict__ bxlo, QArgs29 q,
+                   Fr* __restrict__ T) {
   const size_t n4 = (THREE ? 3 : 4) * n;
   size_t i = (size_t)blockIdx.x * blockDim.x + threadIdx.x;
   if (i >= n4) return;
@@ -567,7 +568,7 @@
     izw = (i + 4) & (n4 - 1);
     cj = (int)(i & 3);
   }
-  const F29 a = split29(A[i]), b = split29(B[i]), c = split29(C[i]), z = split29(Z[i]);
+  const F29 a = split29(A[i]), b = split29(B[i]), c = split29(C[i]);
   F29 gate;
   {
     const F29 ga[4] = {mul29<Fr29>(a, b), a, b, c};
@@ -576,8 +577,10 @@
   }
   if (npub > 0) gate = add29(gate, q29_pi(cl, Apub, 0, npub < 4 ? npub : 4, n4, i));
   if (npub > 4) gate = add29(gate, q29_pi(cl, Apub, 4, npub - 4, n4, i));
-  const F29 x = mul29<Fr29>(split29(xlo[ix & 4095]), split29(xhi[ix >> 12]));
-  const F29 bx = mul29<Fr29>(q.beta, x);
+  const F29 z = split29(Z[i]);
+  const bool bxt = THREE && q.k23;
+  const F29 x = mul29<Fr29>(split29((bxt ? bxlo : xlo)[ix & 4095]), split29(xhi[ix >> 12]));
+  const F29 bx = bxt ? x : mul29<Fr29>(q.beta, x);
   const F29 bx2 = q.k23 ? add29(bx, bx) : mul29<Fr29>(q.bk1, x);
   const F29 bx3 = q.k23 ? add29(bx2, bx) : mul29<Fr29>(q.bk2, x);
   const F29 f1 = add29(add29(a, bx), q.gamma);
@@ -591,7 +594,13 @@
   const F29 pa[2] = {q.alpha, q.alpha2};
   const F29 pb[2] = {sub29(num, den, Fr29::K2), mul29<Fr29>(add29(z, q.negone), split29(cl[i]))};
   const F29 S = add29(gate, mulsum29<Fr29, 2>(pa, pb));
-  T[i] = join_fr29(mul29<Fr29>(S, q.zhinv[cj]));
+  T[i] = THREE ? canon_fr29(S) : join_fr29(mul29<Fr29>(S, q.zhinv[cj]));
+}
+
+__global__ void __launch_bounds__(kT)
+k_beta_xlo(const Fr* __restrict__ xlo, F29 beta, size_t count, Fr* __restrict__ bxlo) {
+  const size_t i = (size_t)blockIdx.x * blockDim.x + threadIdx.x;
+  if (i < count) bxlo[i] = join_fr29(mul29<Fr29>(beta, split29(xlo[i])));
 }
 
 __global__ void __launch_bounds__(kT)
@@ -1071,22 +1080,18 @@
   }
   if (quot3) {
     const size_t nhi3 = (n + 4095) / 4096;
-    tw3.alloc((size_t)3 * n);
+    ctw3.alloc((size_t)3 * (n - 1));
     itw3.alloc((size_t)3 * n);
     const Fr inv4n = inverse(fr_small(n4));
     DevBuf<Fr> lo, hi;
     for (int j = 0; j < 3; j++) {
       const Fr cj = g * pow_u64(w4, (uint64_t)j), cji = inverse(cj);
       d3[j] = pow_u64(cj, n);
-      table(lo, nlo, cj, one);
-      table(hi, nhi3, pow_u64(cj, 4096), one);
-      hipLaunchKernelGGL(k_factor29_table, dim3(grid_for(n, kT, 1u << 30)), dim3(kT), 0, s, tw3.p + (size_t)j * n,
-                         lo.p, hi.p, one, (size_t)n);
-      NZ_HIP(hipStreamSynchronize(s));
+      ntt_coset_twiddles(eng->ntt_tables, cj, power, ctw3.p + (size_t)j * (n - 1), s);
       table(lo, nlo, cji, one);
       table(hi, nhi3, pow_u64(cji, 4096), one);
       hipLaunchKernelGGL(k_factor29_table, dim3(grid_for(n, kT, 1u << 30)), dim3(kT), 0, s, itw3.p + (size_t)j * n,
-                         lo.p, hi.p, inv4n, (size_t)n);
+                         lo.p, hi.p, inv4n * zh_inv[j], (size_t)n);
       NZ_HIP(hipGetLastError());
       NZ_HIP(hipStreamSynchronize(s));
     }
@@ -1103,7 +1108,7 @@
       for (int j = 0; j < 3; j++) {
         NttIo io;
         io.in_len = n;
-        io.in_f = tw3.p + (size_t)j * n;
+        io.tw = ctw3.p + (size_t)j * (n - 1);
         ntt(eng->ntt_tables, coefs, out + (size_t)j * n, power, false, s, nullptr, &io);
       }
     };
@@ -1179,6 +1184,7 @@
   const size_t ne = quot3 ? (size_t)3 * n : n4;
   A4.alloc(ne); B4.alloc(ne); C4.alloc(ne); Z4.alloc(ne);
   T.alloc(ne); Tz.alloc(ne); t.alloc(quot3 ? ne + 6 : n4);
+  if (quot3) bx_lo.alloc(4096);
   pol_r.alloc(n + 3); pol_wxi.alloc(n + 6); pol_wxiw.alloc(n + 3);
   blind.alloc(13);
   scan_tmp.alloc(3 * ((size_t)n / kTileN + 2) + 64);
@@ -1226,7 +1232,7 @@
   cq.alias(pk.cq); cs.alias(pk.cs); cl.alias(pk.cl);
   quot3 = pk.quot3;
   cq3.alias(pk.cq3); cs3.alias(pk.cs3); cl3.alias(pk.cl3);
-  tw3.alias(pk.tw3); itw3.alias(pk.itw3);
+  ctw3.alias(pk.ctw3); itw3.alias(pk.itw3);
   for (int j = 0; j < 3; j++) d3[j] = pk.d3[j];
   std::memcpy(sig_top, pk.sig_top, sizeof(sig_top));
   alloc_workspace();
@@ -1260,8 +1266,10 @@
   q29.gamma = f29_exp(gamma, 0);
   q29.negone = f29_exp(neg(Fr::one()), 0);
   q29.alpha = f29_exp(alpha, 20);
+  if (q29.k23)
+    hipLaunchKernelGGL(k_beta_xlo, dim3(grid_for(4096, kT)), dim3(kT), 0, s, x_lo.p, q29.beta, (size_t)4096, bx_lo.p);
   hipLaunchKernelGGL((k_quotient_coset29<true>), dim3(grid_for(n3, kT, 1u << 30)), dim3(kT), 0, s, A4.p, B4.p, C4.p,
-                     Z4.p, cq3.p, cs3.p, cl3.p, nPublic, A.p, (size_t)n, x_lo.p, root_hi.p, q29, T.p);
+                     Z4.p, cq3.p, cs3.p, cl3.p, nPublic, A.p, (size_t)n, x_lo.p, root_hi.p, bx_lo.p, q29, T.p);
   if (!side) launch_gate_check(s);
   for (int j = 0; j < 3; j++) {
     NttIo io;
@@ -1346,7 +1354,7 @@
     for (int j = 0; j < 3; j++) {
       NttIo io;
       io.in_len = n;
-      io.in_f = tw3.p + (size_t)j * n;
+      io.tw = ctw3.p + (size_t)j * (n - 1);
       io.fold_len = (size_t)nb;
       io.fold_n = n;
       io.fold_f = fr29_operand(d3[j]);
@@ -1824,7 +1832,8 @@
       q29.negone = f29_exp(neg(Fr::one()), 0);
       q29.alpha = f29_exp(alpha, 20);
       hipLaunchKernelGGL((k_quotient_coset29<false>), dim3(grid_for(n4, kT, 1u << 30)), dim3(kT), 0, s, A4.p, B4.p,
-                         C4.p, Z4.p, cq.p, cs.p, cl.p, nPublic, A.p, (size_t)n, x_lo.p, root_hi.p, q29, T.p);
+                         C4.p, Z4.p, cq.p, cs.p, cl.p, nPublic, A.p, (size_t)n, x_lo.p, root_hi.p, (const Fr*)nullptr, q29,
+                         T.p);
     } else {
       hipLaunchKernelGGL(k_quotient_coset, dim3(grid_for(n4, kT, 1u << 30)), dim3(kT), 0, s, A4.p, B4.p, C4.p,
                          Z4.p, cq.p, cs.p, cl.p, nPublic, A.p, (size_t)n, x_lo.p, root_hi.p, q, T.p);
diff --git a/nzcb-circom_amd/nzcb/__init__.py b/nzcb-circom_amd/nzcb/__init__.py
--- a/nzcb-circom_amd/nzcb/__init__.py
+++ b/nzcb-circom_amd/nzcb/__init__.py
@@ -34,6 +34,7 @@
     "nzcb_nzcp_witness_dev", "nzcb_synth_setup_ex", "nzcb_memcpy_d2d",
     "nzcb_plonk_setup", "nzcb_prove_batch_status", "nzcb_wprog_remap", "nzcb_prove_logged", "nzcb_memcpy_d2d_async",
     "nzcb_debug_guard_check", "nzcb_debug_guard_selftest", "nzcb_debug_inject_fault", "nzcb_debug_f29",
+    "nzcb_debug_ntt_coset",
     "nzcb_msm_table_create_lagrange",
     "nzcb_verify_batch", "nzcb_engine_g1_lincomb", "nzcb_engine_verify_batch", "nzcb_debug_verify_batch_timings",
     "nzcb_r1cs_create", "nzcb_r1cs_create_file", "nzcb_r1cs_info", "nzcb_r1cs_check", "nzcb_r1cs_destroy",
@@ -75,7 +76,7 @@
     return checked.value
 
 
-F29_WORDS = {1: (27, 9), 2: (54, 18), 3: (18, 9), 4: (36, 18), 5: (18, 18), 6: (36, 9)}
+F29_WORDS = {1: (27, 9), 2: (54, 18), 3: (18, 9), 4: (36, 18), 5: (18, 18), 6: (36, 9), 7: (10, 9)}
 
 
 def f29_check(op: int, words, device: int = 0):
@@ -188,6 +189,7 @@
         "nzcb_engine_create": (c_void_p, [c_int, c_int, c_size_t, POINTER(_Err)]),
         "nzcb_engine_destroy": (None, [c_void_p]),
         "nzcb_engine_ntt": (c_int, [c_void_p, u8p, u8p, c_int, c_int, POINTER(_Err)]),
+        "nzcb_debug_ntt_coset": (c_int, [c_void_p, u8p, u8p, c_int, u8p, c_int, POINTER(_Err)]),
         "nzcb_engine_msm": (c_int, [c_void_p, u8p, u8p, c_size_t, c_int, u8p, POINTER(_Err)]),
         "nzcb_dev_alloc": (c_void_p, [c_size_t]),
         "nzcb_dev_alloc_on": (c_void_p, [c_int, c_size_t]),
@@ -454,6 +456,16 @@
         _check(self.lib.nzcb_engine_ntt(self.h, _buf(data_lem), out, log_n, int(inverse), ctypes.byref(err)), err)
         return bytes(out)
 
+    def ntt_coset(self, data_lem: bytes, log_n: int, c_lem: bytes) -> bytes:
+        n = 1 << log_n
+        fold = len(data_lem) // 32 - n
+        assert len(data_lem) == 32 * (n + fold) and fold >= 0 and len(c_lem) == 32
+        out = _out(32 * n)
+        err = _Err()
+        _check(self.lib.nzcb_debug_ntt_coset(self.h, _buf(data_lem), out, log_n, _buf(c_lem), fold,
+                                             ctypes.byref(err)), err)
+        return bytes(out)
+
     def msm(self, bases_lem: bytes, scalars: bytes, scalars_mont: bool = False) -> bytes:
         n = len(scalars) // 32
         assert len(bases_lem) == 64 * n
```

Result: faster. 47.84 proofs/s, median of 6 (+1.4%).
